# max-andr/joint-cnn-mrf

Hardware: AMD Instinct MI355X
Metric: images/sec (720x480, K=9 joints) part-detector+spatial-model fwd (higher is better)
Workload: dtype f32(fp16x2 spectra, fft); 1 GPU; configs[1]: batch=64/GPU synthetic 480x720x3, part detector + spatial model forward + argmax, fp32; batch_per_gpu=64, global_batch=64, micro_batch=64, use_sm=True, collective=all_gather coords int32 [B,2,9]

## Files before the change

### joint-cnn-mrf_amd/csrc/conv_fft.hip

```cpp
#include <cmath>
#include <cstdlib>
#include <map>
#include <mutex>
#include <utility>
#include <vector>

#include "conv_fft_common.h"

namespace jcm {
namespace cfft {

template <int KS, int NP>
__global__ __launch_bounds__(256) void weight_spectra_split_kernel(const float* __restrict__ w, uint4* __restrict__ Ws, int Cin, int Cout, int CoutP, int ntl, int NY, int NX,
                                                                   int round_bf16, float* __restrict__ wscale) {
  __shared__ cf twy[192][KS - 1], twx[KS];
  const int tid = threadIdx.x;
  const int kx = blockIdx.y;
#pragma unroll 1
  for (int k = tid; k < NY * (KS - 1) + KS; k += 256) {
    const bool isy = k < NY * (KS - 1);
    const int ky = k / (KS - 1), a = isy ? k % (KS - 1) + 1 : k - NY * (KS - 1);
    const int num = isy ? (ky * a) % NY : (kx * a) % NX, den = isy ? NY : NX;
    double sn, cs;
    sincospi(-2.0 * (double)num / (double)den, &sn, &cs);
    cf* dstw = isy ? &twy[ky][a - 1] : &twx[a];
    *dstw = cf{(float)cs, (float)sn};
  }
  __syncthreads();
  constexpr int CPT = 8;
  constexpr int NPP = NP == 5 ? 1 : 2;
  static_assert(NP == 2 || NP == 4 || NP == 5, "operand forms of the channel GEMM");
  float wmul = 1.f;
  if constexpr (NP >= 4) {
    int ex = 0;
    const float bound = wscale[0];
    if (bound > 0.f && bound < 3.0e38f) (void)frexpf(bound, &ex);
    wmul = ldexpf(1.f, 14 - ex);
    if (blockIdx.x == 0 && blockIdx.y == 0 && threadIdx.x == 0) wscale[1] = ldexpf(1.f, ex - 14);
  }
  const size_t e = (size_t)blockIdx.x * 256 + tid;
  if (e >= (size_t)(Cin / CPT) * CoutP) return;
  const int co = (int)(e % CoutP), cig = (int)(e / CoutP);
  cf ra[CPT][KS];
  const unsigned toff = (unsigned)(cig * CPT * Cout + (co < Cout ? co : Cout - 1));
#pragma unroll
  for (int c = 0; c < CPT; ++c)
#pragma unroll
    for (int a = 0; a < KS; ++a) ra[c][a] = cf{0.f, 0.f};
#pragma unroll 1
  for (int a = 0; a < KS; ++a) {
    cf sum[CPT];
#pragma unroll
    for (int c = 0; c < CPT; ++c) sum[c] = cf{0.f, 0.f};
#pragma unroll
    for (int b = 0; b < KS; ++b) {
      const float* tap = w + (size_t)((KS - 1 - a) * KS + (KS - 1 - b)) * Cin * Cout;
      const cf tw = twx[b];
#pragma unroll
      for (int c = 0; c < CPT; ++c) {
        float wv = tap[toff + (unsigned)(c * Cout)];
        wv = co < Cout ? wv : 0.f;
        if (round_bf16) wv = static_cast<float>(static_cast<__bf16>(wv));
        sum[c] = sfma(wv, tw, sum[c]);
      }
    }
#pragma unroll
    for (int c = 0; c < CPT; ++c)
#pragma unroll
      for (int aa = 0; aa < KS; ++aa) ra[c][aa] = aa == a ? sum[c] : ra[c][aa];
  }
  const int KC = Cin / 16, ntiles = CoutP / ntl;
  const int ci0 = cig * CPT, kc = ci0 >> 4, kg = (ci0 >> 3) & 1, nt = co / ntl, sn = co % ntl;
  const size_t fstride = NP == 5 ? (size_t)ntiles * (KC >> 1) * 8 * ntl : (size_t)ntiles * KC * (4 * NPP) * ntl;
  uint4* dst = Ws + (size_t)kx * NY * fstride +
               (NP == 5 ? ((size_t)nt * (KC >> 1) + (kc >> 1)) * 8 * ntl + ((size_t)(kc & 1) * 2 + kg) * ntl + sn :
                          ((size_t)nt * KC + kc) * (4 * NPP) * ntl + (size_t)kg * ntl + sn);
  typedef unsigned u32x4n __attribute__((ext_vector_type(4)));
  auto put = [](uint4* q, const uint4& v) __attribute__((always_inline)) { __builtin_nontemporal_store(u32x4n{v.x, v.y, v.z, v.w}, reinterpret_cast<u32x4n*>(q)); };
  auto emit = [&](uint4* d, const float (&xr)[CPT], const float (&xi)[CPT]) __attribute__((always_inline)) {
    if constexpr (NP == 5) {
      float x8[8];
#pragma unroll
      for (int c = 0; c < 8; ++c) x8[c] = xr[c % CPT];
      put(d, round8h(x8, wmul));
#pragma unroll
      for (int c = 0; c < 8; ++c) x8[c] = xi[c % CPT];
      put(d + (size_t)4 * ntl, round8h(x8, wmul));
    } else {
      uint4 u[NPP];
      float x8[8];
#pragma unroll
      for (int c = 0; c < 8; ++c) x8[c] = xr[c % CPT];
      if constexpr (NP == 4) split8h(x8, wmul, u);
      else split8<NPP>(x8, u);
#pragma unroll
      for (int p = 0; p < NPP; ++p) put(d + (size_t)p * 2 * ntl, u[p]);
#pragma unroll
      for (int c = 0; c < 8; ++c) x8[c] = xi[c % CPT];
      if constexpr (NP == 4) split8h(x8, wmul, u);
      else split8<NPP>(x8, u);
#pragma unroll
      for (int p = 0; p < NPP; ++p) put(d + (size_t)(NPP + p) * 2 * ntl, u[p]);
    }
  };
  for (int ky = 0; ky <= NY / 2; ++ky) {
    const int kp = ky == 0 ? 0 : NY - ky;
    float cs[KS - 1], sn_[KS - 1];
#pragma unroll
    for (int a = 1; a < KS; ++a) { const cf t = twy[ky][a - 1]; cs[a - 1] = t.x; sn_[a - 1] = -t.y; }
    float xr[CPT], xi[CPT], pr[CPT], pi_[CPT];
#pragma unroll
    for (int c = 0; c < CPT; ++c) {
      cf C = ra[c][0], S = cf{0.f, 0.f};
#pragma unroll
      for (int a = 1; a < KS; ++a) { C = sfma(cs[a - 1], ra[c][a], C); S = sfma(sn_[a - 1], ra[c][a], S); }
      xr[c] = C.x + S.y; xi[c] = C.y - S.x;
      pr[c] = C.x - S.y; pi_[c] = C.y + S.x;
    }
    emit(dst + (size_t)ky * fstride, xr, xi);
    if (kp != ky) emit(dst + (size_t)kp * fstride, pr, pi_);
  }
}

template <int TAPS>
__global__ __launch_bounds__(256) void weight_bound_kernel(const float* __restrict__ w, size_t pairs, int round_bf16, float* __restrict__ wmax) {
  __shared__ float red[4];
  float m = 0.f;
  for (size_t e = (size_t)blockIdx.x * 256 + threadIdx.x; e < pairs; e += (size_t)gridDim.x * 256) {
    float v[TAPS];
#pragma unroll
    for (int t = 0; t < TAPS; ++t) v[t] = w[(size_t)t * pairs + e];
    float sum = 0.f;
#pragma unroll
    for (int t = 0; t < TAPS; ++t) {
      float x = v[t];
      if (round_bf16) x = static_cast<float>(static_cast<__bf16>(x));
      sum += fabsf(x);
    }
    m = fmaxf(m, sum);
  }
  block_max_to<256>(m * 1.0001f, wmax, red, threadIdx.x);
}

struct Sizes { int NY, NX; };
static const int kLens[] = {20, 24, 28, 32, 36, 40, 50, 60, 64, 72, 96, 100, 128, 192};
static bool pick(int need, int* n) {
  for (int v : kLens)
    if (v >= need) { *n = v; return true; }
  return false;
}
static int tw_offset(int n) {
  int off = 0;
  for (int v : kLens) {
    if (v == n) return off;
    off += v;
  }
  return -1;
}
static bool sizes_of(int H, int W, int ks, Sizes* s, int circ = 0) {
  if (circ) {
    s->NY = H; s->NX = W;
    return (ks == 9 || ks == 5) && H > 8 && W > 8 && tw_offset(H) >= 0 && tw_offset(W) >= 0;
  }
  return (ks == 9 || ks == 5) && H + ks - 1 <= 192 && W + ks - 1 <= 192 && pick(H + 4, &s->NY) && pick(W + 4, &s->NX);
}
static int pad64(int c) { return (c + CB - 1) / CB * CB; }
static bool fft_reg_on() {
  static const bool on = [] { const char* e = std::getenv("JCM_FFT_REG"); return !e || std::atoi(e) != 0; }();
  return on;
}
static bool fft_tiles_on() {
  static const bool on = [] { const char* e = std::getenv("JCM_FFT_TILES"); return !e || std::atoi(e) != 0; }();
  return on;
}
static int padn(int c, int n) { return (c + n - 1) / n * n; }

int persistent_grid(const void* kernel, int ntiles, int threads, int dyn_lds) {
  static std::mutex mu;
  static std::map<std::pair<const void*, int>, int> cache;
  int dev = 0;
  (void)hipGetDevice(&dev);
  int resident = 0;
  {
    std::lock_guard<std::mutex> lk(mu);
    auto it = cache.find({kernel, dev});
    if (it != cache.end()) resident = it->second;
  }
  if (!resident) {
    int ncu = 256, per_cu = 0;
    (void)hipDeviceGetAttribute(&ncu, hipDeviceAttributeMultiprocessorCount, dev);
    if (hipOccupancyMaxActiveBlocksPerMultiprocessor(&per_cu, kernel, threads, (size_t)dyn_lds) != hipSuccess || per_cu < 1) per_cu = 1;
    resident = ncu * per_cu;
    std::lock_guard<std::mutex> lk(mu);
    cache[{kernel, dev}] = resident;
  }
  return resident < ntiles ? resident : ntiles;
}

static const cf* twiddle_table(int dev) {
  static std::mutex mu;
  static std::map<int, cf*> tabs;
  std::lock_guard<std::mutex> lk(mu);
  auto it = tabs.find(dev);
  if (it != tabs.end()) return it->second;
  std::vector<float> h;
  for (int n : kLens)
    for (int k = 0; k < n; ++k) {
      const double ang = 2.0 * 3.14159265358979323846 * (double)k / (double)n;
      h.push_back((float)std::cos(ang));
      h.push_back((float)std::sin(ang));
    }
  cf* d = nullptr;
  if (hipMalloc(reinterpret_cast<void**>(&d), h.size() * sizeof(float)) != hipSuccess) return nullptr;
  if (hipMemcpy(d, h.data(), h.size() * sizeof(float), hipMemcpyHostToDevice) != hipSuccess) { (void)hipFree(d); return nullptr; }
  tabs[dev] = d;
  return d;
}

}

using namespace cfft;

bool conv_fft_supported(const ConvArgs& a, int ks) {
  Sizes s;
  return a.Cin % CB == 0 && a.Cin >= CB && a.Cout >= 1 && a.B >= 1 && sizes_of(a.H, a.W, ks, &s, a.circ);
}
size_t conv_fft_weight_bytes(int H, int W, int ks, int Cin, int Cout, int np, int circ) {
  Sizes s;
  if (!sizes_of(H, W, ks, &s, circ)) return 0;
  return cgemm_split_w_bytes(np, s.NY * (s.NX / 2 + 1), Cin, Cout);
}
hipError_t conv_fft_pack_weights(const float* w_hwio, void* wf, int H, int W, int ks, int Cin, int Cout, int np, bool round_bf16, hipStream_t st, float* wscale, int circ,
                                 const float* bound_from) {
  Sizes s;
  if (!sizes_of(H, W, ks, &s, circ) || Cin % 16 || (np != 2 && np != 4 && np != 5) || (np >= 4 && !wscale) || (np == 5 && Cin % 32)) return hipErrorInvalidValue;
  const int ntl = cgemm_split_ntile(np, Cout), CoutP = padn(Cout, ntl);
  const size_t cpt = 8;
  const dim3 grid((unsigned)(((size_t)Cin / cpt * CoutP + 255) / 256), (unsigned)(s.NX / 2 + 1));
  uint4* dst = static_cast<uint4*>(wf);
  const int rb = round_bf16 ? 1 : 0;
  if (np >= 4 && bound_from) {
    if (hipError_t e = hipMemcpyAsync(wscale, bound_from, sizeof(float), hipMemcpyDeviceToDevice, st); e != hipSuccess) return e;
  } else if (np >= 4) {
    if (hipError_t e = hipMemsetAsync(wscale, 0, 2 * sizeof(float), st); e != hipSuccess) return e;
    const size_t pairs = (size_t)Cin * Cout;
    const dim3 bgrid((unsigned)((pairs + 255) / 256 > 1024 ? 1024 : (pairs + 255) / 256));
    if (ks == 9) hipLaunchKernelGGL(weight_bound_kernel<81>, bgrid, dim3(256), 0, st, w_hwio, pairs, rb, wscale);
    else hipLaunchKernelGGL(weight_bound_kernel<25>, bgrid, dim3(256), 0, st, w_hwio, pairs, rb, wscale);
  }
#define WS_LAUNCH(KS, NPV) hipLaunchKernelGGL((weight_spectra_split_kernel<KS, NPV>), grid, dim3(256), 0, st, w_hwio, dst, Cin, Cout, CoutP, ntl, s.NY, s.NX, rb, wscale)
  if (ks == 9) {
    if (np == 2) WS_LAUNCH(9, 2); else if (np == 4) WS_LAUNCH(9, 4); else WS_LAUNCH(9, 5);
  } else {
    if (np == 2) WS_LAUNCH(5, 2); else if (np == 4) WS_LAUNCH(5, 4); else WS_LAUNCH(5, 5);
  }
#undef WS_LAUNCH
  return hipGetLastError();
}
namespace {
struct Plan3 { size_t t_bytes, xs_bytes, yf_bytes, sc_fwd_bytes, sc_inv_bytes; int MT, NXH, F, ldy, inv_cb; };
Plan3 plan_of(const ConvArgs& a, const Sizes& s, int np) {
  Plan3 p;
  p.NXH = s.NX / 2 + 1;
  p.F = s.NY * p.NXH;
  p.ldy = padn(a.Cout, cgemm_split_ntile(np, a.Cout));
  if (p.ldy < pad64(a.Cout)) p.ldy = pad64(a.Cout);
  p.MT = cgemm_split_mtile(np, a.B, a.Cout);
  const size_t cop = pad64(a.Cout), cmax = (size_t)a.Cin > cop ? a.Cin : cop;
  const size_t bp = (size_t)(a.B + p.MT - 1) / p.MT * p.MT;
  p.t_bytes = (size_t)a.B * p.NXH * a.H * cmax * sizeof(cf);
  p.xs_bytes = (size_t)p.F * bp * a.Cin * 4 * cgemm_split_parts(np);
  p.yf_bytes = (size_t)p.F * a.B * p.ldy * sizeof(cf);
  p.inv_cb = s.NY > 100 ? 32 : 64;
  p.sc_fwd_bytes = (size_t)a.B * a.H * (a.Cin / CB) * sizeof(float);
  p.sc_inv_bytes = (size_t)a.B * p.NXH * (cop / p.inv_cb) * sizeof(float);
  return p;
}
size_t align256(size_t v) { return (v + 255) & ~size_t(255); }
ConvArgs tile_view(const ConvArgs& a, const Sizes& s) {
  ConvArgs t = a;
  t.B = 4 * a.B; t.H = s.NY; t.W = a.W / 2;
  t.tiles = 0;
  return t;
}
}
size_t conv_fft_workspace_bytes(const ConvArgs& a, int ks, int np) {
  Sizes s;
  if (!(a.tiles ? sizes_of(a.H / 2, a.W / 2, ks, &s) : sizes_of(a.H, a.W, ks, &s, a.circ))) return 0;
  const Plan3 p = a.tiles ? plan_of(tile_view(a, s), s, np) : plan_of(a, s, np);
  return align256(p.t_bytes) + align256(p.xs_bytes) + align256(p.yf_bytes) + align256(p.sc_fwd_bytes) + align256(p.sc_inv_bytes);
}
bool conv_fft_fusable(const ConvArgs& a, int ks, int ks_next) {
  Sizes s, n;
  return sizes_of(a.H, a.W, ks, &s) && sizes_of(a.H, a.W, ks_next, &n) && s.NX == n.NX && a.Cout % CB == 0;
}
size_t conv_fft_handover_bytes(const ConvArgs& a, int ks) {
  Sizes s;
  if (!sizes_of(a.H, a.W, ks, &s)) return 0;
  return (size_t)a.B * (s.NX / 2 + 1) * a.H * a.Cout * sizeof(cf);
}
bool conv_fft_win_gather_supported(int win, int Cin) { return fft_reg_on() && cfft_rows_fwd_win_reg_supported(win, Cin); }
bool conv_fft_win_scatter_supported(int win, int Cout) { return fft_reg_on() && win == 32 && Cout % 64 == 0; }
bool conv_fft_pool_fusable(const ConvArgs& a, int ks, int ks_next) {
  Sizes s, n;
  return sizes_of(a.H, a.W, ks, &s) && sizes_of((a.H + 1) / 2, (a.W + 1) / 2, ks_next, &n) && cfft_rows_inv_pool_fwd_supported(s.NX, n.NX, a.Cout);
}
size_t conv_fft_pool_handover_bytes(const ConvArgs& a, int ks_next) {
  Sizes n;
  if (!sizes_of((a.H + 1) / 2, (a.W + 1) / 2, ks_next, &n)) return 0;
  return (size_t)a.B * (n.NX / 2 + 1) * ((a.H + 1) / 2) * a.Cout * sizeof(cf);
}
bool conv_fft_tiles_supported(const ConvArgs& a, int ks, int ks_next) {
  Sizes s;
  return fft_reg_on() && fft_tiles_on() && ks == 5 && ks_next == 5 && !a.circ && !a.win_map && a.B >= 1 && conv_fft_pool_fusable(a, ks, ks_next) &&
         a.H % 4 == 0 && a.W % 4 == 0 && sizes_of(a.H / 2, a.W / 2, ks, &s) && cfft_tiles_supported(s.NY, s.NX, a);
}
bool conv_fft_merge_fusable(const ConvArgs& a, int ks, int ks_next, const FftMerge& m, bool h16) {
  Sizes s;
  if (!conv_fft_fusable(a, ks, ks_next) || !sizes_of(a.H, a.W, ks, &s)) return false;
  const bool reg = fft_reg_on() && cfft_rows_inv_merge_fwd_reg_supported(s.NX, a, m, (ks - 1) / 2);
  return h16 ? reg : (reg || cfft_rows_inv_merge_fwd_supported(s.NX, a, m));
}
static hipError_t conv_fft_tiles_f32(const ConvArgs& a0, int ks, int np, int in_layout, void* work, const void* t_in, void* t_next, const FftMerge* merge,
                                     hipEvent_t g0, hipEvent_t g1, hipStream_t st, void* xs, bool xs_ready, const Fp16Scale* scp, const FftNext* nx) {
  Sizes s;
  if (np != 4 || in_layout != 0 || t_in || merge || xs || xs_ready || !t_next || !nx || !nx->pool || nx->merge || !scp || !scp->tmax || !scp->winv || !scp->tmax_next ||
      !conv_fft_tiles_supported(a0, ks, nx->ks_next) || !sizes_of(a0.H / 2, a0.W / 2, ks, &s))
    return hipErrorInvalidValue;
  ConvArgs a = a0;
  a.CoutP = pad64(a.Cout);
  const ConvArgs at = tile_view(a, s);
  const Plan3 p = plan_of(at, s, np);
  Fp16Scale sc = *scp;
  sc.hf = (float)s.NY;
  sc.nb = at.B;
  char* wk = static_cast<char*>(work);
  cf* T = reinterpret_cast<cf*>(wk);
  void* Xs = wk + align256(p.t_bytes);
  cf* Yf = reinterpret_cast<cf*>(wk + align256(p.t_bytes) + align256(p.xs_bytes));
  int dev = 0;
  if (hipError_t e = hipGetDevice(&dev); e != hipSuccess) return e;
  const cf* twb = twiddle_table(dev);
  if (!twb) return hipErrorOutOfMemory;
  if (!cfft_rows_fwd_tile_reg(s.NY, s.NX, a, T, sc.tmax, st)) return hipErrorInvalidValue;
  if (hipError_t ce = cfft_cols_fwd(s.NY, at, np, T, Xs, twb + tw_offset(s.NY), p.NXH, p.MT, sc, st); ce != hipSuccess) return ce;
  if (hipError_t e = hipGetLastError(); e != hipSuccess) return e;
  if (g0 && hipEventRecord(g0, st) != hipSuccess) return hipErrorUnknown;
  if (hipError_t e = cgemm_split(Xs, a.wp, Yf, np, p.F, at.B, a.Cin, a.Cout, p.ldy, st, 0.f); e != hipSuccess) return e;
  if (g1 && hipEventRecord(g1, st) != hipSuccess) return hipErrorUnknown;
  ConvArgs ai = at;
  ai.H = a.H / 2;
  if (!cfft_cols_inv_reg(s.NY, ai, Yf, T, p.NXH, p.ldy, (ks - 1) / 2, st, nullptr, 0.f)) return hipErrorInvalidValue;
  if (!cfft_rows_inv_pool_tile_reg(s.NY, s.NX, a, T, static_cast<cf*>(t_next), 1.0f / (float)(s.NY * s.NX), sc, st)) return hipErrorInvalidValue;
  return hipGetLastError();
}
hipError_t conv_fft_f32(const ConvArgs& a0, int ks, int np, int in_layout, int out_layout, void* work, const void* t_in, void* t_next, const FftMerge* merge,
                        hipEvent_t g0, hipEvent_t g1, hipStream_t st, void* xs, bool xs_ready, const Fp16Scale* scp, const FftNext* nx) {
  if (a0.tiles) return conv_fft_tiles_f32(a0, ks, np, in_layout, work, t_in, t_next, merge, g0, g1, st, xs, xs_ready, scp, nx);
  Sizes s;
  if (!conv_fft_supported(a0, ks) || !sizes_of(a0.H, a0.W, ks, &s, a0.circ) || (out_layout == 2 && a0.Cout % 8) || (np != 2 && np != 4 && np != 5) || (np == 5 && a0.Cin % 32)) return hipErrorInvalidValue;
  if (a0.circ && (t_in || t_next || merge || in_layout != 0 || out_layout != 0)) return hipErrorInvalidValue;
  if (nx && (nx->pool || nx->merge) && (!t_next || (nx->pool && nx->merge))) return hipErrorInvalidValue;
  Fp16Scale sc;
  if (np >= 4) {
    if (!scp || !scp->tmax || !scp->winv || (t_next && !scp->tmax_next)) return hipErrorInvalidValue;
    sc = *scp;
    sc.hf = (float)a0.H;
    sc.nb = a0.B;
  }
  const bool h16 = sc.t16 && ((t_next && nx && nx->merge && !t_in) || (t_in && !t_next));
  if ((t_in || t_next) && !h16 && (in_layout != 0 || out_layout != 0)) return hipErrorInvalidValue;
  if (t_next && a0.Cout % CB) return hipErrorInvalidValue;
  if (sc.t16 && (np != 5 || in_layout == 0 || out_layout == 0 || xs || ((t_in || t_next) && !h16))) return hipErrorInvalidValue;
  if (merge && in_layout == 2) return hipErrorInvalidValue;
  ConvArgs a = a0;
  a.CoutP = pad64(a.Cout);
  const int opad = (ks - 1) / 2 + (a0.circ ? 4 : 0);
  const Plan3 p = plan_of(a, s, np);
  char* wk = static_cast<char*>(work);
  cf* T = reinterpret_cast<cf*>(wk);
  void* Xs = xs ? xs : wk + align256(p.t_bytes);
  cf* Yf = reinterpret_cast<cf*>(wk + align256(p.t_bytes) + align256(p.xs_bytes));
  if (sc.t16) {
    sc.t16_fwd = reinterpret_cast<float*>(wk + align256(p.t_bytes) + align256(p.xs_bytes) + align256(p.yf_bytes));
    sc.t16_inv = reinterpret_cast<float*>(wk + align256(p.t_bytes) + align256(p.xs_bytes) + align256(p.yf_bytes) + align256(p.sc_fwd_bytes));
    sc.t16_cb = p.inv_cb;
    if (t_in) sc.t16_fwd = reinterpret_cast<float*>(const_cast<char*>(static_cast<const char*>(t_in)) + align256((size_t)a.B * p.NXH * a.H * a.Cin * 4));
  }
  if (xs_ready && !xs) return hipErrorInvalidValue;
  int dev = 0;
  if (hipError_t e = hipGetDevice(&dev); e != hipSuccess) return e;
  const cf* twb = twiddle_table(dev);
  if (!twb) return hipErrorOutOfMemory;
  const cf* twx = twb + tw_offset(s.NX);
  const cf* twy = twb + tw_offset(s.NY);
  const float norm = 1.0f / (float)(s.NY * s.NX);
  const cf* Tin = t_in ? static_cast<const cf*>(t_in) : T;
  const bool fft_reg = fft_reg_on();
  if (!xs_ready) {
    if (merge && !t_in) {
      if (!(fft_reg && cfft_rows_fwd_merge_reg(s.NX, a, *merge, in_layout, T, sc.tmax, st, sc.t16_fwd))) cfft_rows_fwd_merge(s.NX, a, *merge, in_layout, T, twx, sc.tmax, st, sc.t16_fwd);
    } else if (!t_in) {
      if (a.win_map) { if (!cfft_rows_fwd_win_reg(s.NX, a, T, sc.tmax, st)) return hipErrorInvalidValue; }
      else if (!(fft_reg && cfft_rows_fwd_reg(s.NX, a, in_layout, T, sc.tmax, st, sc.t16_fwd))) cfft_rows_fwd(s.NX, a, in_layout, T, twx, sc.tmax, st, sc.t16_fwd);
    }
    if (hipError_t ce = cfft_cols_fwd(s.NY, a, np, Tin, Xs, twy, p.NXH, p.MT, sc, st); ce != hipSuccess) return ce;
  }
  if (hipError_t e = hipGetLastError(); e != hipSuccess) return e;
  if (g0 && hipEventRecord(g0, st) != hipSuccess) return hipErrorUnknown;
  const float yshift = sc.t16 ? cgemm_split_y16_shift(a.Cin) : 0.f, yinv = yshift != 0.f ? 1.0f / yshift : 0.f;
  if (hipError_t e = cgemm_split(Xs, a.wp, Yf, np, p.F, a.B, a.Cin, a.Cout, p.ldy, st, yshift); e != hipSuccess) return e;
  if (g1 && hipEventRecord(g1, st) != hipSuccess) return hipErrorUnknown;
  ConvArgs ai = a;
  if (a0.circ) { ai.H = a0.H - 8; ai.W = a0.W - 8; }
  if (!(fft_reg && p.inv_cb == 64 && cfft_cols_inv_reg(s.NY, ai, Yf, T, p.NXH, p.ldy, opad, st, sc.t16_inv, yinv))) cfft_cols_inv(s.NY, ai, Yf, T, twy, p.NXH, p.ldy, opad, st, sc.t16_inv, yinv);
  if (t_next && nx && nx->pool) {
    Sizes sn;
    if (!sizes_of((a.H + 1) / 2, (a.W + 1) / 2, nx->ks_next, &sn) ||
        !cfft_rows_inv_pool_fwd(s.NX, sn.NX, a, T, static_cast<cf*>(t_next), twx, twb + tw_offset(sn.NX), opad, norm, sc, st))
      return hipErrorInvalidValue;
  } else if (t_next && nx && nx->merge) {
    if (sc.t16) {
      float* t16n = reinterpret_cast<float*>(static_cast<char*>(t_next) + align256((size_t)a.B * p.NXH * a.H * a.Cout * 4));
      if (!(fft_reg && cfft_rows_inv_merge_fwd_reg(s.NX, a, *nx->merge, T, static_cast<cf*>(t_next), opad, norm, sc, st, t16n))) return hipErrorInvalidValue;
    } else if (!(fft_reg && cfft_rows_inv_merge_fwd_reg(s.NX, a, *nx->merge, T, static_cast<cf*>(t_next), opad, norm, sc, st)) &&
               !cfft_rows_inv_merge_fwd(s.NX, a, *nx->merge, T, static_cast<cf*>(t_next), twx, opad, norm, sc, st)) {
      return hipErrorInvalidValue;
    }
  } else if (t_next) {
    if (!(fft_reg && cfft_rows_inv_fwd_reg(s.NX, a, T, static_cast<cf*>(t_next), opad, norm, sc, st))) cfft_rows_inv_fwd(s.NX, a, T, static_cast<cf*>(t_next), twx, opad, norm, sc, st);
  } else if (!((ai.rows_mfma & 1) && cfft_rows_inv_mfma(s.NX, ai, out_layout, T, opad, norm, sc, st)) && !(fft_reg && cfft_rows_inv_reg(s.NX, ai, out_layout, T, opad, norm, sc, st))) {
    if (ai.wout_TX > 0) return hipErrorInvalidValue;
    cfft_rows_inv(s.NX, ai, out_layout, T, twx, opad, norm, sc, st);
  }
  return hipGetLastError();
}

size_t conv_fft_xs_bytes(const ConvArgs& a, int ks, int np) {
  Sizes s;
  if (!sizes_of(a.H, a.W, ks, &s, a.circ)) return 0;
  return align256(plan_of(a, s, np).xs_bytes);
}
hipError_t conv_fft_spectra(const ConvArgs& a0, int ks, int np, void* work, void* xs, hipStream_t st, float* tmax, int common) {
  Sizes s;
  if (!conv_fft_supported(a0, ks) || !sizes_of(a0.H, a0.W, ks, &s, a0.circ) || !xs || (np >= 4 && !tmax)) return hipErrorInvalidValue;
  Fp16Scale sc;
  if (np >= 4) { sc.tmax = tmax; sc.hf = (float)a0.H; sc.nb = a0.B; sc.common = common; }
  ConvArgs a = a0;
  a.CoutP = pad64(a.Cout);
  const Plan3 p = plan_of(a, s, np);
  int dev = 0;
  if (hipError_t e = hipGetDevice(&dev); e != hipSuccess) return e;
  const cf* twb = twiddle_table(dev);
  if (!twb) return hipErrorOutOfMemory;
  cf* T = static_cast<cf*>(work);
  if (a.win_map) { if (!cfft_rows_fwd_win_reg(s.NX, a, T, sc.tmax, st)) return hipErrorInvalidValue; }
  else cfft_rows_fwd(s.NX, a, 0, T, twb + tw_offset(s.NX), sc.tmax, st);
  if (hipError_t ce = cfft_cols_fwd(s.NY, a, np, T, xs, twb + tw_offset(s.NY), p.NXH, p.MT, sc, st); ce != hipSuccess) return ce;
  return hipGetLastError();
}
bool conv_fft_geometry(int H, int W, int ks, int B, int Cout, int np, int* NY, int* NX, int* MT, int circ) {
  Sizes s;
  if (!sizes_of(H, W, ks, &s, circ)) return false;
  *NY = s.NY; *NX = s.NX; *MT = cgemm_split_mtile(np, B, Cout);
  return true;
}

}
```

### joint-cnn-mrf_amd/csrc/conv_fft_cols.hip

```cpp
#include "conv_fft_common.h"

namespace jcm {
namespace cfft {

template <int NY, int NP, bool T16 = false>
__global__ __launch_bounds__(colfwd_threads<NY>()) void cols_fwd_split_kernel(const cf* __restrict__ T, uint4* __restrict__ Xs, const cf* __restrict__ twg, int B, int H, int KC, int MT,
                                                            int mtiles, const float* __restrict__ tmax, int common, const float* __restrict__ t16, int ntiles) {
  constexpr int IMG = colimg<NY>(), CH = IMG * 16, NTC = colfwd_threads<NY>(), NPP = NP == 5 ? 1 : 2;
  constexpr int CPV = T16 ? 4 : 2;
  constexpr int NV = NY * CH / CPV, KV = (NV + NTC - 1) / NTC, VPR = CH / CPV, VPI = 16 / CPV;
  extern __shared__ __attribute__((aligned(16))) char smem_cf[];
  cf* buf = reinterpret_cast<cf*>(smem_cf);
  cf* tw = buf + NY * CH;
  float4* buf4 = reinterpret_cast<float4*>(buf);
  const int tid = threadIdx.x;
  const int NG = (B + IMG - 1) / IMG;
  twiddles<NY, NTC>(tw, twg, tid);
  __shared__ float xsc[IMG];
  uint4 pre[KV];
  float psc[KV];
  auto coords = [&](int tile, int& kc, int& kx, int& b0, int& nimg) __attribute__((always_inline)) {
    const int g = tile % NG, kk = tile / NG;
    kc = kk % KC; kx = kk / KC;
    b0 = g * IMG; nimg = min(IMG, B - b0);
  };
  auto prefetch = [&](int tile) __attribute__((always_inline)) {
    int kc, kx, b0, nimg;
    coords(tile, kc, kx, b0, nimg);
    const uint4* src = reinterpret_cast<const uint4*>(T) + (((size_t)kx * KC + kc) * B + b0) * H * VPI;
#pragma unroll
    for (int i = 0; i < KV; ++i) {
      const int t = tid + i * NTC, y = t / VPR, v = t % VPR, img = v / VPI, cv = v % VPI;
      const bool ok = t < NV && y < H && img < nimg;
      pre[i] = ok ? src[((size_t)img * H + y) * VPI + cv] : make_uint4(0u, 0u, 0u, 0u);
      if constexpr (T16) psc[i] = ok ? t16[((size_t)(b0 + img) * (KC >> 2) + (kc >> 2)) * H + y] : 0.f;
    }
  };
  int tile = blockIdx.x;
  if (tile < ntiles) prefetch(tile);
  for (; tile < ntiles; tile += gridDim.x) {
    int kc, kx, b0, nimg;
    coords(tile, kc, kx, b0, nimg);
#pragma unroll
    for (int i = 0; i < KV; ++i) {
      const int t = tid + i * NTC;
      if (t < NV) {
        if constexpr (T16) {
          const cf a = unpack_h2(pre[i].x, psc[i]), b2 = unpack_h2(pre[i].y, psc[i]), c2 = unpack_h2(pre[i].z, psc[i]), d2 = unpack_h2(pre[i].w, psc[i]);
          buf4[2 * t] = make_float4(a.x, a.y, b2.x, b2.y);
          buf4[2 * t + 1] = make_float4(c2.x, c2.y, d2.x, d2.y);
        } else {
          buf4[t] = make_float4(__uint_as_float(pre[i].x), __uint_as_float(pre[i].y), __uint_as_float(pre[i].z), __uint_as_float(pre[i].w));
        }
      }
    }
    if constexpr (NP >= 4)
      if (tid < IMG) xsc[tid] = tid < nimg ? fp16_scale(tmax_of(tmax, b0 + tid, B, common), (float)H) : 1.f;
    __syncthreads();
    if (tile + (int)gridDim.x < ntiles) prefetch(tile + (int)gridDim.x);
    fft<NY, -1, CH, NTC>(buf, tw, tid);
    const int mt = b0 / MT, r0 = b0 - mt * MT;
    for (int it = tid; it < NY * 2 * IMG; it += NTC) {
      const int img = it % IMG, kg = (it / IMG) & 1, ky = it / (2 * IMG);
      const cf* z = buf + pos<NY>(ky) * CH + img * 16 + kg * 8;
      float re[8], im[8];
#pragma unroll
      for (int e = 0; e < 8; ++e) { re[e] = z[e].x; im[e] = z[e].y; }
      uint4 ur[NPP], ui[NPP];
      if constexpr (NP == 5) {
        const float xscale = xsc[img];
        ur[0] = round8h(re, xscale);
        ui[0] = round8h(im, xscale);
      } else if constexpr (NP == 4) {
        const float xscale = xsc[img];
        split8h(re, xscale, ur);
        split8h(im, xscale, ui);
      } else {
        split8<NPP>(re, ur);
        split8<NPP>(im, ui);
      }
      const size_t f = (size_t)kx * NY + ky;
      if constexpr (NP == 5) {
        uint4* dst = Xs + (((f * mtiles + mt) * (KC >> 1) + (kc >> 1)) * 8 + (size_t)(kc & 1) * 2 + kg) * MT + r0 + img;
        st_stream(dst, ur[0]);
        st_stream(dst + (size_t)4 * MT, ui[0]);
      } else {
        uint4* dst = Xs + (((f * mtiles + mt) * KC + kc) * (4 * NPP) + kg) * MT + r0 + img;
#pragma unroll
        for (int p = 0; p < NPP; ++p) {
          st_stream(dst + (size_t)(0 * NPP + p) * 2 * MT, ur[p]);
          st_stream(dst + (size_t)(1 * NPP + p) * 2 * MT, ui[p]);
        }
      }
    }
    __syncthreads();
  }
}

template <int NY, bool T16 = false>
__global__ __launch_bounds__(colinv_threads<NY>()) void cols_inv_kernel(const cf* __restrict__ Yf, cf* __restrict__ T, const cf* __restrict__ twg, int B, int H, int NXH, int C, int ldy,
                                                      int pad, float* __restrict__ t16, float yinv) {
  constexpr int CH = colblk<NY>(), CB = CH, NTC = colinv_threads<NY>();
  __shared__ cf buf[NY * CH];
  __shared__ cf tw[NY];
  const int tid = threadIdx.x;
  const int cblk = blockIdx.x % (C / CB), bk = blockIdx.x / (C / CB);
  const int kx = bk % NXH, b = bk / NXH;
  twiddles<NY, NTC>(tw, twg, tid);
  for (int t = tid; t < NY * CH; t += NTC) {
    const int ky = t / CH, v = t % CH;
    const size_t src = ((size_t)(kx * NY + ky) * B + b) * ldy + cblk * CB + v;
    if constexpr (T16) buf[t] = unpack_h2(reinterpret_cast<const unsigned*>(Yf)[src], 1.f);
    else buf[t] = Yf[src];
  }
  __syncthreads();
  fft<NY, 1, CH, NTC>(buf, tw, tid);
  if constexpr (T16) {
    constexpr int KM = (NY * CH + NTC - 1) / NTC;
    __shared__ float red[NTC / 64];
    cf val[KM];
    float m = 0.f;
#pragma unroll
    for (int i = 0; i < KM; ++i) {
      const int t = tid + i * NTC, y = t / CH, v = t % CH;
      val[i] = cf{0.f, 0.f};
      if (t < H * CH) {
        val[i] = buf[pos<NY>(y + pad) * CH + v];
        m = fmaxf(m, fmaxf(fabsf(val[i].x), fabsf(val[i].y)));
      }
    }
    const float s = bfp_scale(block_max_all<NTC>(m, red, tid));
    unsigned* dst = reinterpret_cast<unsigned*>(T);
#pragma unroll
    for (int i = 0; i < KM; ++i) {
      const int t = tid + i * NTC, y = t / CH, v = t % CH;
      if (t < H * CH) st_stream(&dst[((size_t)(b * H + y) * NXH + kx) * C + cblk * CB + v], pack_h2(val[i].x * s, val[i].y * s));
    }
    if (tid == 0) t16[((size_t)b * (C / CB) + cblk) * NXH + kx] = (1.0f / s) * yinv;
  } else {
    for (int t = tid; t < H * CH; t += NTC) {
      const int y = t / CH, v = t % CH;
      st_stream(&T[((size_t)(b * H + y) * NXH + kx) * C + cblk * CB + v], buf[pos<NY>(y + pad) * CH + v]);
    }
  }
}


template <int NY> static hipError_t launch_cols_fwd(const ConvArgs& a, int np, const cf* T, void* Xs, const cf* tw, int NXH, int MT, const Fp16Scale& sc, hipStream_t st) {
  constexpr int IMG = colimg<NY>();
  constexpr int lds = (NY * IMG * 16 + NY) * (int)sizeof(cf);
  const int KC = a.Cin / 16, mtiles = (a.B + MT - 1) / MT;
  const int ntiles = NXH * KC * ((a.B + IMG - 1) / IMG);
  static LdsAttr attr2, attr4, attr5, attr5h;
  const dim3 blk(colfwd_threads<NY>());
#define COLS_FWD(KERNEL, ATTR, ...)                                                                              \
  do {                                                                                                           \
    if (hipError_t e = ATTR.ensure(reinterpret_cast<const void*>(KERNEL), lds); e != hipSuccess) return e;        \
    const dim3 grid((unsigned)persistent_grid(reinterpret_cast<const void*>(KERNEL), ntiles, (int)blk.x, lds));  \
    hipLaunchKernelGGL(KERNEL, grid, blk, lds, st, T, static_cast<uint4*>(Xs), tw, a.B, a.H, KC, MT, mtiles, __VA_ARGS__, ntiles); \
  } while (0)
  if (np == 5 && sc.t16_fwd) {
    if (!sc.tmax || (KC & 3)) return hipErrorInvalidValue;
    COLS_FWD((cols_fwd_split_kernel<NY, 5, true>), attr5h, sc.tmax, sc.common, sc.t16_fwd);
  } else if (np == 5) {
    if (!sc.tmax || (KC & 1)) return hipErrorInvalidValue;
    COLS_FWD((cols_fwd_split_kernel<NY, 5>), attr5, sc.tmax, sc.common, (const float*)nullptr);
  } else if (np == 2) {
    COLS_FWD((cols_fwd_split_kernel<NY, 2>), attr2, (const float*)nullptr, 0, (const float*)nullptr);
  } else if (np == 4) {
    if (!sc.tmax) return hipErrorInvalidValue;
    COLS_FWD((cols_fwd_split_kernel<NY, 4>), attr4, sc.tmax, sc.common, (const float*)nullptr);
  } else {
    return hipErrorInvalidValue;
  }
#undef COLS_FWD
  return hipSuccess;
}
template <int NY> static void launch_cols_inv(const ConvArgs& a, const cf* Yf, cf* T, const cf* tw, int NXH, int ldy, int pad, hipStream_t st, float* t16, float y16_inv) {
  const dim3 grid(a.B * NXH * (a.CoutP / colblk<NY>())), blk(colinv_threads<NY>());
  if (t16) hipLaunchKernelGGL((cols_inv_kernel<NY, true>), grid, blk, 0, st, Yf, T, tw, a.B, a.H, NXH, a.CoutP, ldy, pad, t16, y16_inv);
  else hipLaunchKernelGGL((cols_inv_kernel<NY, false>), grid, blk, 0, st, Yf, T, tw, a.B, a.H, NXH, a.CoutP, ldy, pad, nullptr, 0.f);
}
hipError_t cfft_cols_fwd(int NY, const ConvArgs& a, int np, const cf* T, void* Xs, const cf* tw, int NXH, int MT, const Fp16Scale& sc, hipStream_t st) {
  hipError_t e = hipSuccess;
#define CALL(N) e = launch_cols_fwd<N>(a, np, T, Xs, tw, NXH, MT, sc, st)
  CFFT_BY_SIZE(NY, CALL)
#undef CALL
  return e;
}
void cfft_cols_inv(int NY, const ConvArgs& a, const cf* Yf, cf* T, const cf* tw, int NXH, int ldy, int pad, hipStream_t st, float* t16, float y16_inv) {
#define CALL(N) launch_cols_inv<N>(a, Yf, T, tw, NXH, ldy, pad, st, t16, y16_inv)
  CFFT_BY_SIZE(NY, CALL)
#undef CALL
}

}
}
```

### joint-cnn-mrf_amd/csrc/conv_fft_common.h

```cpp
#pragma once
#include "fft_lds.h"
#include "kernels.h"

namespace jcm {
namespace cfft {
using namespace fftl;
constexpr int CB = 64, NT = 256;
constexpr int kParMax = 512;

template <int N> struct Plan;
template <> struct Plan<192> { static constexpr int R1 = 8, R2 = 8, R3 = 3; };
template <> struct Plan<128> { static constexpr int R1 = 8, R2 = 4, R3 = 4; };
template <> struct Plan<100> { static constexpr int R1 = 4, R2 = 5, R3 = 5; };
template <> struct Plan<96> { static constexpr int R1 = 8, R2 = 12, R3 = 1; };
template <> struct Plan<72> { static constexpr int R1 = 8, R2 = 3, R3 = 3; };
template <> struct Plan<64> { static constexpr int R1 = 8, R2 = 8, R3 = 1; };
template <> struct Plan<60> { static constexpr int R1 = 4, R2 = 15, R3 = 1; };
template <> struct Plan<50> { static constexpr int R1 = 5, R2 = 10, R3 = 1; };
template <> struct Plan<40> { static constexpr int R1 = 8, R2 = 5, R3 = 1; };
template <> struct Plan<36> { static constexpr int R1 = 4, R2 = 3, R3 = 3; };
template <> struct Plan<32> { static constexpr int R1 = 8, R2 = 4, R3 = 1; };
template <> struct Plan<28> { static constexpr int R1 = 4, R2 = 7, R3 = 1; };
template <> struct Plan<24> { static constexpr int R1 = 8, R2 = 3, R3 = 1; };
template <> struct Plan<20> { static constexpr int R1 = 4, R2 = 5, R3 = 1; };
// ... 84 lines not shown
  return ((((size_t)k * (C >> 4) + cblk * 4 + (v >> 3)) * B + b) * H + y) * 8 + (v & 7);
}
template <int NX, int NTH = NT>
__device__ __forceinline__ float rows_fwd_store(const cf* buf, cf* __restrict__ T, int tid, int cblk, int b, int y, int B, int H, int C) {
  constexpr int CH = CB / 2, NXH = NX / 2 + 1;
  float4* dst = reinterpret_cast<float4*>(T);
  float m = 0.f;
  for (int t = tid; t < NXH * CH; t += NTH) {
    const int k = t / CH, v = t % CH;
    const cf zk = buf[pos<NX>(k) * CH + v], zn = buf[pos<NX>(k == 0 ? 0 : NX - k) * CH + v];
    const float4 o = make_float4(0.5f * (zk.x + zn.x), 0.5f * (zk.y - zn.y), 0.5f * (zk.y + zn.y), -0.5f * (zk.x - zn.x));
    dst[t_fwd_index(k, cblk, v, b, y, B, H, C)] = o;
    m = fmaxf(fmaxf(m, fmaxf(fabsf(o.x), fabsf(o.y))), fmaxf(fabsf(o.z), fabsf(o.w)));
  }
  return m;
}

template <int NX, int NTH = NT>
__device__ __forceinline__ float rows_fwd_store16(const cf* buf, void* T, float* __restrict__ tinv, float* red2, int tid, int cblk, int b, int y, int B, int H, int C) {
  constexpr int CH = CB / 2, NXH = NX / 2 + 1, K = (NXH * CH + NTH - 1) / NTH;
  uint2* dst = reinterpret_cast<uint2*>(T);
  float4 o[K];
  float m = 0.f;
#pragma unroll
  for (int i = 0; i < K; ++i) {
    const int t = tid + i * NTH, k = t / CH, v = t % CH;
    o[i] = make_float4(0.f, 0.f, 0.f, 0.f);
    if (t < NXH * CH) {
      const cf zk = buf[pos<NX>(k) * CH + v], zn = buf[pos<NX>(k == 0 ? 0 : NX - k) * CH + v];
      o[i] = make_float4(0.5f * (zk.x + zn.x), 0.5f * (zk.y - zn.y), 0.5f * (zk.y + zn.y), -0.5f * (zk.x - zn.x));
      m = fmaxf(fmaxf(m, fmaxf(fabsf(o[i].x), fabsf(o[i].y))), fmaxf(fabsf(o[i].z), fabsf(o[i].w)));
    }
  }
  const float s = bfp_scale(block_max_all<NTH>(m, red2, tid));
#pragma unroll
  for (int i = 0; i < K; ++i) {
    const int t = tid + i * NTH, k = t / CH, v = t % CH;
    if (t < NXH * CH) dst[t_fwd_index(k, cblk, v, b, y, B, H, C)] = make_uint2(pack_h2(o[i].x * s, o[i].y * s), pack_h2(o[i].z * s, o[i].w * s));
  }
  if (tid == 0) tinv[((size_t)b * (C / CB) + cblk) * H + y] = 1.0f / s;
  return m;
}

constexpr int kFp16TargetExp = 15;
static_assert(kFp16TargetExp <= 15, "sqrt(2) * 2^kFp16TargetExp must stay below fp16's largest number 65504");
__device__ __forceinline__ int fp16_exp(float tmax, float hf) {
  const float bound = tmax * hf;
  int e = 0;
  if (bound > 0.f && bound < 3.0e38f) (void)frexpf(bound, &e);
  return e;
}
__device__ __forceinline__ int fp16_k(float tmax, float hf) { const int k = kFp16TargetExp - fp16_exp(tmax, hf); return k > 126 ? 126 : (k < -126 ? -126 : k); }
__device__ __forceinline__ float fp16_scale(float tmax, float hf) { return ldexpf(1.f, fp16_k(tmax, hf)); }
__device__ __forceinline__ float fp16_unscale(float tmax, float hf) { return ldexpf(1.f, -fp16_k(tmax, hf)); }
__device__ __forceinline__ float tmax_of(const float* __restrict__ tmax, int b, int nb, int common) {
  if (!common) return tmax[b];
  float m = 0.f;
  for (int i = 0; i < nb; ++i) m = fmaxf(m, tmax[i]);
  return m;
}
__device__ __forceinline__ void wave_max_stash(float m, float* red) {
#pragma unroll
  for (int o = 32; o > 0; o >>= 1) m = fmaxf(m, __shfl_xor(m, o));
  if ((threadIdx.x & 63) == 0) red[threadIdx.x >> 6] = m;
}
template <int NTH>
__device__ __forceinline__ void stash_to_word(const float* red, float* dst) {
  if (threadIdx.x == 0) {
    float m = red[0];
#pragma unroll
    for (int w = 1; w < NTH / 64; ++w) m = fmaxf(m, red[w]);
    if (m > 0.f) atomicMax(reinterpret_cast<unsigned*>(dst), __float_as_uint(m));
  }
}
template <int NTH>
__device__ __forceinline__ void block_max_to(float m, float* dst, float* red, int tid) {
#pragma unroll
  for (int o = 32; o > 0; o >>= 1) m = fmaxf(m, __shfl_xor(m, o));
  if ((tid & 63) == 0) red[tid >> 6] = m;
  __syncthreads();
  if (tid == 0) {
    for (int w = 1; w < NTH / 64; ++w) m = fmaxf(m, red[w]);
    if (m > 0.f) atomicMax(reinterpret_cast<unsigned*>(dst), __float_as_uint(m));
  }
}
template <int NX> constexpr int rows_threads() { return NX >= 128 ? 512 : NX >= 72 ? 384 : 256; }
template <int NY> constexpr int colblk() { return NY > 100 ? 32 : 64; }
template <int NY> constexpr int colimg() { return NY > 96 ? 4 : 8; }
template <int NY> constexpr int colfwd_threads() { return NY * colimg<NY>() * 16 >= 8192 ? 1024 : NY * colimg<NY>() * 16 >= 4096 ? 512 : 256; }
template <int NY> constexpr int colinv_threads() { return NY * colblk<NY>() >= 4096 ? 512 : 256; }
__device__ __forceinline__ void split8h(const float (&x)[8], float scale, uint4 (&out)[2]) {
  unsigned short h[2][8];
#pragma unroll
  for (int e = 0; e < 8; ++e) {
    float v = x[e] * scale;
#pragma unroll
    for (int p = 0; p < 2; ++p) {
      const _Float16 q = static_cast<_Float16>(v);
      h[p][e] = __builtin_bit_cast(unsigned short, q);
      v = v - static_cast<float>(q);
    }
  }
#pragma unroll
  for (int p = 0; p < 2; ++p)
    out[p] = make_uint4((unsigned)h[p][0] | ((unsigned)h[p][1] << 16), (unsigned)h[p][2] | ((unsigned)h[p][3] << 16), (unsigned)h[p][4] | ((unsigned)h[p][5] << 16),
                        (unsigned)h[p][6] | ((unsigned)h[p][7] << 16));
}
__device__ __forceinline__ uint4 round8h(const float (&x)[8], float scale) {
  unsigned short h[8];
#pragma unroll
  for (int e = 0; e < 8; ++e) h[e] = __builtin_bit_cast(unsigned short, static_cast<_Float16>(x[e] * scale));
  return make_uint4((unsigned)h[0] | ((unsigned)h[1] << 16), (unsigned)h[2] | ((unsigned)h[3] << 16), (unsigned)h[4] | ((unsigned)h[5] << 16), (unsigned)h[6] | ((unsigned)h[7] << 16));
}
template <int NP>
__device__ __forceinline__ void split8(const float (&x)[8], uint4 (&out)[NP]) {
  unsigned short h[NP][8];
#pragma unroll
  for (int e = 0; e < 8; ++e) {
    float v = x[e];
#pragma unroll
    for (int p = 0; p < NP; ++p) {
      const __bf16 q = static_cast<__bf16>(v);
      h[p][e] = __builtin_bit_cast(unsigned short, q);
      v = v - static_cast<float>(q);
    }
  }
#pragma unroll
  for (int p = 0; p < NP; ++p)
    out[p] = make_uint4((unsigned)h[p][0] | ((unsigned)h[p][1] << 16), (unsigned)h[p][2] | ((unsigned)h[p][3] << 16), (unsigned)h[p][4] | ((unsigned)h[p][5] << 16),
                        (unsigned)h[p][6] | ((unsigned)h[p][7] << 16));
}
#define CFFT_BY_SIZE(N, CALL)                    \
  switch (N) {                                   \
    case 20: CALL(20); break;                    \
    case 24: CALL(24); break;                    \
    case 28: CALL(28); break;                    \
    case 32: CALL(32); break;                    \
    case 36: CALL(36); break;                    \
    case 40: CALL(40); break;                    \
    case 50: CALL(50); break;                    \
    case 60: CALL(60); break;                    \
    case 64: CALL(64); break;                    \
    case 72: CALL(72); break;                    \
    case 96: CALL(96); break;                    \
    case 100: CALL(100); break;                  \
    case 128: CALL(128); break;                  \
    default: CALL(192); break;                   \
  }

int persistent_grid(const void* kernel, int ntiles, int threads, int dyn_lds = 0);

void cfft_rows_fwd(int NX, const ConvArgs& a, int layout, cf* T, const cf* tw, float* tmax, hipStream_t st, float* t16 = nullptr);
void cfft_rows_fwd_merge(int NX, const ConvArgs& a, const FftMerge& m, int in_layout, cf* T, const cf* tw, float* tmax, hipStream_t st, float* t16 = nullptr);
hipError_t cfft_cols_fwd(int NY, const ConvArgs& a, int np, const cf* T, void* Xs, const cf* tw, int NXH, int MT, const Fp16Scale& sc, hipStream_t st);
void cfft_cols_inv(int NY, const ConvArgs& a, const cf* Yf, cf* T, const cf* tw, int NXH, int ldy, int pad, hipStream_t st, float* t16 = nullptr, float y16_inv = 0.f);
void cfft_rows_inv(int NX, const ConvArgs& a, int layout, const cf* T, const cf* tw, int pad, float norm, const Fp16Scale& sc, hipStream_t st);
bool cfft_rows_inv_reg(int NX, const ConvArgs& a, int layout, const cf* T, int pad, float norm, const Fp16Scale& sc, hipStream_t st);
bool cfft_rows_inv_fwd_reg(int NX, const ConvArgs& a, const cf* T, cf* Tn, int pad, float norm, const Fp16Scale& sc, hipStream_t st);
bool cfft_rows_fwd_reg(int NX, const ConvArgs& a, int layout, cf* T, float* tmax, hipStream_t st, float* t16);
bool cfft_rows_fwd_win_reg(int NX, const ConvArgs& a, cf* T, float* tmax, hipStream_t st);
bool cfft_rows_fwd_win_reg_supported(int NX, int Cin);
bool cfft_tiles_supported(int NY, int NX, const ConvArgs& a);
bool cfft_rows_fwd_tile_reg(int NY, int NX, const ConvArgs& a, cf* T, float* tmax, hipStream_t st);
bool cfft_rows_inv_pool_tile_reg(int NY, int NX, const ConvArgs& a, const cf* T, cf* Tn, float norm, const Fp16Scale& sc, hipStream_t st);
bool cfft_rows_fwd_merge_reg(int NX, const ConvArgs& a, const FftMerge& m, int in_layout, cf* T, float* tmax, hipStream_t st, float* t16);
bool cfft_cols_inv_reg(int NY, const ConvArgs& a, const cf* Yf, cf* T, int NXH, int ldy, int pad, hipStream_t st, float* t16, float y16_inv = 0.f);
void cfft_rows_inv_fwd(int NX, const ConvArgs& a, const cf* T, cf* Tn, const cf* tw, int pad, float norm, const Fp16Scale& sc, hipStream_t st);
bool cfft_rows_inv_pool_fwd(int NXI, int NXO, const ConvArgs& a, const cf* T, cf* Tn, const cf* twi, const cf* two, int pad, float norm, const Fp16Scale& sc, hipStream_t st);
bool cfft_rows_inv_merge_fwd(int NX, const ConvArgs& a, const FftMerge& m, const cf* T, cf* Tn, const cf* tw, int pad, float norm, const Fp16Scale& sc, hipStream_t st);
bool cfft_rows_inv_merge_fwd_reg(int NX, const ConvArgs& a, const FftMerge& m, const cf* T, cf* Tn, int pad, float norm, const Fp16Scale& sc, hipStream_t st, float* t16n = nullptr);
bool cfft_rows_inv_merge_fwd_reg_supported(int NX, const ConvArgs& a, const FftMerge& m, int pad);
bool cfft_rows_inv_pool_fwd_supported(int NXI, int NXO, int Cout);
bool cfft_rows_inv_mfma(int NX, const ConvArgs& a, int layout, const cf* T, int pad, float norm, const Fp16Scale& sc, hipStream_t st);
bool cfft_rows_inv_merge_fwd_supported(int NX, const ConvArgs& a, const FftMerge& m);
}
}
```

### joint-cnn-mrf_amd/csrc/conv_fft_rows_reg.hip

```cpp
#include <type_traits>

#include "conv_fft_common.h"
#include "fft_reg.h"
#include "resize_tf1.h"

namespace jcm {
namespace cfft {
using namespace fftr;

template <int NX, int K1, bool ALL = false, class St>
__device__ __forceinline__ void inv_rows_out2(const cf (&u)[NX / 2], int h, int W, int pad, St&& store) {
  constexpr int M = NX / 2, R1 = RPlan<M>::R1, R2 = RPlan<M>::R2;
  cf o[R2];
  step2_row<M, 1, K1>(u, o);
#pragma unroll
  for (int k2 = 0; k2 < R2; ++k2) {
    const int xo = 2 * (K1 + R1 * k2) + h - pad;
    if (ALL || (xo >= 0 && xo < W)) store(K1 + R1 * k2, xo, o[k2]);
  }
  __builtin_amdgcn_sched_barrier(0);
  if constexpr (K1 + 1 < R1) inv_rows_out2<NX, K1 + 1, ALL>(u, h, W, pad, store);
}
template <int NX, int N>
__device__ __forceinline__ void inv_rows_in2(cf (&u)[NX / 2], const float4& q1, const float4& q2, float sg, bool odd) {
// ... 65 lines not shown
      typedef float f4 __attribute__((ext_vector_type(4)));
      const f4 q = __builtin_bit_cast(f4, __builtin_amdgcn_raw_buffer_load_b128(d, vo, k * ko, 0));
      return make_float4(q[0], q[1], q[2], q[3]);
    };
    inv_rows_load2<NX, T16, 0>(u, sg, odd, load);
  }
  float norm = norm0;
  if (sc.tmax) {
    float tm;
    if (sc.common) {
      tm = 0.f;
      for (int i = (int)(threadIdx.x & 63); i < sc.nb; i += 64) tm = fmaxf(tm, sc.tmax[i]);
#pragma unroll
      for (int o = 32; o > 0; o >>= 1) tm = fmaxf(tm, __shfl_xor(tm, o));
    } else {
      tm = sc.tmax[b];
    }
    norm = norm0 * sc.winv[0] * fp16_unscale(tm, sc.hf);
  }
  const bool two = c + 1 < Cout;
  float b0v = 0.f, b1v = 0.f, s0 = 1.f, s1 = 1.f, h0 = 0.f, h1 = 0.f;
  if (c < Cout) {
    b0v = bias[c];
    if (two) b1v = bias[c + 1];
    if (relu_bn) { s0 = scale[c]; h0 = shift[c]; if (two) { s1 = scale[c + 1]; h1 = shift[c + 1]; } }
  }
  step1<M, 1>(u);
  const int lane = threadIdx.x & 63;
  int sc_row = -1, sc_x0 = 0;
  if (LAYOUT == 0 && sTX > 0) {
    const int bw = (int)(by / H), yv = (int)(by % H);
    const int tx = bw % sTX, ty = (bw / sTX) % sTY, bi = bw / (sTX * sTY), ym = ty * H + yv;
    sc_row = ym < smH ? bi * smH + ym : -1;
    sc_x0 = tx * W;
  }
  unsigned* wst = stage + (LAYOUT != 0 ? (threadIdx.x >> 6) * (M * 64) : 0);
  auto store = [&](int m, int xo, cf z) __attribute__((always_inline)) {
    float v0 = fmaf(z.x, norm, b0v), v1 = fmaf(z.y, norm, b1v);
    if (relu_bn) { v0 = fmaf(fmaxf(v0, 0.f), s0, h0); v1 = fmaf(fmaxf(v1, 0.f), s1, h1); }
    if constexpr (LAYOUT == 0) {
      if (sTX > 0) {
        const int xm = sc_x0 + xo;
        if (sc_row >= 0 && xm < smW) st_stream(reinterpret_cast<cf*>(static_cast<float*>(out) + ((size_t)sc_row * smW + xm) * Cout + c), cf{v0, v1});
      } else {
        st_stream(reinterpret_cast<cf*>(static_cast<float*>(out) + (by * W + xo) * Cout + c), cf{v0, v1});
      }
    } else {
      typedef __bf16 bf16x2 __attribute__((ext_vector_type(2)));
      wst[(m * 2 + h) * 32 + (lane >> 1)] = __builtin_bit_cast(unsigned, bf16x2{static_cast<__bf16>(v0), static_cast<__bf16>(v1)});
    }
  };
  if (two || LAYOUT != 0) inv_rows_out2<NX, 0, LAYOUT != 0>(u, h, W, pad, store);
  if constexpr (LAYOUT != 0) {
    __builtin_amdgcn_fence(__ATOMIC_RELEASE, "wavefront");
    __builtin_amdgcn_wave_barrier();
    const int y = (int)(by % H);
    const int c0 = c - (lane >> 1) * 2;
    const uint4* rd = reinterpret_cast<const uint4*>(wst);
#pragma unroll 4
    for (int q = lane; q < M * 16; q += 64) {
      const int m = q >> 4, hh = (q >> 3) & 1, j = q & 7;
      const int xo = 2 * m + hh - pad, cu = c0 + 8 * j;
      if (xo >= 0 && xo < W && cu < Cout) {
        __bf16* o = LAYOUT == 1 ? static_cast<__bf16*>(out) + (by * W + xo) * Cout + cu
                                : static_cast<__bf16*>(out) + (((size_t)b * (Cout >> 3) + (cu >> 3)) * H * W + (size_t)y * W + xo) * 8;
        *reinterpret_cast<uint4*>(o) = rd[q];
      }
    }
  }
}

template <int NY, int K1>
__device__ __forceinline__ void inv_cols_rows(cf (&x)[NY]) {
  constexpr int R1 = RPlan<NY>::R1, R2 = RPlan<NY>::R2;
  cf o[R2];
  step2_row<NY, 1, K1>(x, o);
#pragma unroll
  for (int k2 = 0; k2 < R2; ++k2) x[R2 * K1 + k2] = o[k2];
  if constexpr (K1 + 1 < R1) inv_cols_rows<NY, K1 + 1>(x);
}
__device__ __forceinline__ unsigned lane_pair_swap(unsigned w) { return (unsigned)__builtin_amdgcn_mov_dpp((int)w, 0xB1, 0xF, 0xF, true); }
template <int NY, bool T16>
__global__ __launch_bounds__(256) __attribute__((amdgpu_waves_per_eu(NY >= 64 ? 2 : 3, NY >= 64 ? 2 : 8))) void cols_inv_reg_kernel(const cf* __restrict__ Yf, void* __restrict__ T, int B, int H, int NXH, int C, int ldy,
                                                                                              int pad, float* __restrict__ t16, float yinv) {
  static_assert(NY % 2 == 0, "ky pairs");
  constexpr int R1 = RPlan<NY>::R1, R2 = RPlan<NY>::R2;
  const size_t g = (size_t)blockIdx.x * 256 + threadIdx.x;
  const int c = (int)(g % C);
  const unsigned bk = (unsigned)__builtin_amdgcn_readfirstlane((int)(g / C));
  const int kx = (int)(bk % (unsigned)NXH), b = (int)(bk / (unsigned)NXH);
  if (b >= B) return;
  const bool odd = (c & 1) != 0;
  cf x[NY];
  if constexpr (T16) {
    const uint2* src = reinterpret_cast<const uint2*>(reinterpret_cast<const unsigned*>(Yf) + ((size_t)kx * NY * B + b) * ldy + (c & ~1));
    const size_t kstep = (size_t)B * ldy / 2;
    uint2 raw[NY / 2];
#pragma unroll
    for (int i = 0; i < NY / 2; ++i) raw[i] = src[(size_t)(2 * i + (odd ? 1 : 0)) * kstep];
    __builtin_amdgcn_sched_barrier(0);
#pragma unroll
    for (int i = 0; i < NY / 2; ++i) {
      const unsigned keep = odd ? raw[i].y : raw[i].x, recv = lane_pair_swap(odd ? raw[i].x : raw[i].y);
      x[2 * i] = unpack_h2(odd ? recv : keep, 1.f);
      x[2 * i + 1] = unpack_h2(odd ? keep : recv, 1.f);
    }
  } else {
    const cf* src = Yf + ((size_t)kx * NY * B + b) * ldy + c;
#pragma unroll
    for (int ky = 0; ky < NY; ++ky) x[ky] = src[(size_t)ky * B * ldy];
  }
  step1<NY, 1>(x);
  inv_cols_rows<NY, 0>(x);
  if constexpr (T16) {
    float m = 0.f;
#pragma unroll
    for (int i = 0; i < NY; ++i) {
      const int y = (i / R2) + R1 * (i % R2) - pad;
      if (y >= 0 && y < H) m = fmaxf(m, fmaxf(fabsf(x[i].x), fabsf(x[i].y)));
    }
#pragma unroll
    for (int o = 32; o > 0; o >>= 1) m = fmaxf(m, __shfl_xor(m, o));
    const float s = bfp_scale(m);
    if ((threadIdx.x & 63) == 0) t16[((size_t)b * (C >> 6) + (c >> 6)) * NXH + kx] = (1.0f / s) * yinv;
    uint2* dst = reinterpret_cast<uint2*>(reinterpret_cast<unsigned*>(T) + ((size_t)b * H * NXH + kx) * C + (c & ~1));
    const size_t ystep = (size_t)NXH * C / 2;
#pragma unroll
    for (int k = 0; k < NY; k += 2) {
      const int ia = R2 * (k % R1) + k / R1, ib = R2 * ((k + 1) % R1) + (k + 1) / R1;
      const unsigned va = pack_h2(x[ia].x * s, x[ia].y * s), vb = pack_h2(x[ib].x * s, x[ib].y * s);
      const unsigned recv = lane_pair_swap(odd ? va : vb);
      const int y = k - pad + (odd ? 1 : 0);
      if (y >= 0 && y < H) st_stream(dst + (size_t)y * ystep, make_uint2(odd ? recv : va, odd ? vb : recv));
    }
  } else {
#pragma unroll
    for (int i = 0; i < NY; ++i) {
      const int y = (i / R2) + R1 * (i % R2) - pad;
      if (y >= 0 && y < H) st_stream(reinterpret_cast<cf*>(T) + ((size_t)(b * H + y) * NXH + kx) * C + c, x[i]);
    }
  }
}
bool cfft_cols_inv_reg(int NY, const ConvArgs& a, const cf* Yf, cf* T, int NXH, int ldy, int pad, hipStream_t st, float* t16, float y16_inv) {
  if (a.CoutP % 64 || ((y16_inv != 0.f) != (t16 != nullptr)) || (t16 && ldy % 2)) return false;
  const size_t threads = (size_t)a.B * NXH * a.CoutP;
  const dim3 grid((unsigned)((threads + 255) / 256)), blk(256);
#define CI_LAUNCH(N)                                                                                                                                             \
  do {                                                                                                                                                           \
    if (t16) hipLaunchKernelGGL((cols_inv_reg_kernel<N, true>), grid, blk, 0, st, Yf, static_cast<void*>(T), a.B, a.H, NXH, a.CoutP, ldy, pad, t16, y16_inv);            \
    else hipLaunchKernelGGL((cols_inv_reg_kernel<N, false>), grid, blk, 0, st, Yf, static_cast<void*>(T), a.B, a.H, NXH, a.CoutP, ldy, pad, nullptr, 0.f);          \
  } while (0)
  switch (NY) {
    case 64: CI_LAUNCH(64); break;
    case 36: CI_LAUNCH(36); break;
    case 32: CI_LAUNCH(32); break;
    case 20: CI_LAUNCH(20); break;
    default: return false;
  }
#undef CI_LAUNCH
  return true;
}

__device__ __forceinline__ unsigned pair_word(unsigned w, bool odd) {
  const auto r = __builtin_amdgcn_permlane32_swap(w, w, false, false);
  return odd ? r[0] : r[1];
}
__device__ __forceinline__ void pair_coords(int CP, int& h, int& p, size_t& by) {
  const size_t g = (size_t)blockIdx.x * 256 + threadIdx.x;
  const int lane = threadIdx.x & 63;
  const size_t q = (g >> 6) * 32;
  h = lane >> 5;
  p = (int)((q + (lane & 31)) % CP);
  by = (size_t)(unsigned)__builtin_amdgcn_readfirstlane((int)(q / CP));
}
template <int NX, int J>
__device__ __forceinline__ void fwd_rows_in2(cf (&u)[NX / 2], const unsigned (&raw)[NX / 2], float sg, bool odd) {
  constexpr int M = NX / 2;
  const unsigned oth = pair_word(raw[J], odd);
  const cf a = bf16pair(raw[J]), o = bf16pair(oth);
  cf v = cf{fmaf(sg, a.x, o.x), fmaf(sg, a.y, o.y)};
  if constexpr (J > 0) {
    const float wr = odd ? Tw<-J, NX>::re : 1.f, wi = odd ? Tw<-J, NX>::im : 0.f;
    v = cf{fmaf(-v.y, wi, v.x * wr), fmaf(v.x, wi, v.y * wr)};
  }
  u[J] = v;
  if constexpr (J + 1 < M) fwd_rows_in2<NX, J + 1>(u, raw, sg, odd);
}
template <int N, int S, int K1>
__device__ __forceinline__ void step2_inplace(cf (&x)[N]) {
  constexpr int R1 = RPlan<N>::R1, R2 = RPlan<N>::R2;
  cf o[R2];
  step2_row<N, S, K1>(x, o);
#pragma unroll
  for (int k2 = 0; k2 < R2; ++k2) x[R2 * K1 + k2] = o[k2];
  if constexpr (K1 + 1 < R1) step2_inplace<N, S, K1 + 1>(x);
}
template <int NX, int MI, class F>
__device__ __forceinline__ void fwd_rows_visit(const cf (&u)[NX / 2], bool odd, F&& f) {
  constexpr int M = NX / 2, R1 = RPlan<M>::R1, R2 = RPlan<M>::R2;
  constexpr int m0 = (M - MI) % M, m1 = M - 1 - MI;
  const cf zk = u[R2 * (MI % R1) + MI / R1], za = u[R2 * (m0 % R1) + m0 / R1], zb = u[R2 * (m1 % R1) + m1 / R1];
  const cf zn = cf{odd ? zb.x : za.x, odd ? zb.y : za.y};
  f(MI, make_float4(0.5f * (zk.x + zn.x), 0.5f * (zk.y - zn.y), 0.5f * (zk.y + zn.y), -0.5f * (zk.x - zn.x)));
  if constexpr (2 * (MI + 1) <= M) fwd_rows_visit<NX, MI + 1>(u, odd, f);
}
template <int NX>
__device__ __forceinline__ void fwd_rows_finish(const unsigned (&raw)[NX / 2], uint2* __restrict__ T, int h, int p, int b, int y, int B, int H, int C, float* __restrict__ tmax,
                                                float* __restrict__ t16) {
  constexpr int M = NX / 2;
  const bool odd = h != 0;
  const int lane = threadIdx.x & 63;
  cf u[M];
  fwd_rows_in2<NX, 0>(u, raw, odd ? -1.f : 1.f, odd);
  step1<M, -1>(u);
  step2_inplace<M, -1, 0>(u);
  float m = 0.f;
  fwd_rows_visit<NX, 0>(u, odd, [&](int mi, const float4& o) __attribute__((always_inline)) {
    if (2 * mi + h <= M) m = fmaxf(fmaxf(m, fmaxf(fabsf(o.x), fabsf(o.y))), fmaxf(fabsf(o.z), fabsf(o.w)));
  });
#pragma unroll
  for (int sft = 32; sft > 0; sft >>= 1) m = fmaxf(m, __shfl_xor(m, sft));
  const float sc = bfp_scale(m);
  const int cblk = p >> 5, v = p & 31;
  if (lane == 0) {
    t16[((size_t)b * (C >> 6) + cblk) * H + y] = 1.0f / sc;
    if (tmax && m > 0.f) atomicMax(reinterpret_cast<unsigned*>(tmax + b), __float_as_uint(m));
  }
  uint2* dst = T + ((((size_t)cblk * 4 + (v >> 3)) * B + b) * H + y) * 8 + (v & 7);
  const size_t kstride = (size_t)(C >> 4) * B * H * 8;
  fwd_rows_visit<NX, 0>(u, odd, [&](int mi, const float4& o) __attribute__((always_inline)) {
    const int k = 2 * mi + h;
    if (k <= M) dst[(size_t)k * kstride] = make_uint2(pack_h2(o.x * sc, o.y * sc), pack_h2(o.z * sc, o.w * sc));
  });
}
template <int NX>
__global__ __launch_bounds__(256) __attribute__((amdgpu_waves_per_eu(NX >= 96 ? 3 : 4, NX >= 96 ? 3 : 8))) void rows_fwd_reg_kernel(const unsigned* __restrict__ in, uint2* __restrict__ T, int nrows, int B, int H, int W, int C,
                                                                                              float* __restrict__ tmax, float* __restrict__ t16) {
  constexpr int M = NX / 2;
  const int CP = C >> 1;
  int h, p;
  size_t by;
  pair_coords(CP, h, p, by);
  if (by >= (size_t)nrows) return;
  const int b = (int)(by / H), y = (int)(by % H);
  const unsigned* src = in + (by * W) * CP + p;
  unsigned raw[M];
#pragma unroll
  for (int j = 0; j < M; ++j) {
    const int n = h * M + j;
    raw[j] = n < W ? src[(size_t)n * CP] : 0u;
  }
  fwd_rows_finish<NX>(raw, T, h, p, b, y, B, H, C, tmax, t16);
}
bool cfft_rows_fwd_reg(int NX, const ConvArgs& a, int layout, cf* T, float* tmax, hipStream_t st, float* t16) {
  if ((NX != 96 && NX != 50 && NX != 28) || layout != 1 || !t16 || a.Cin % 64 || a.W > NX) return false;
  const int nrows = a.B * a.H;
  const size_t threads = (size_t)nrows * a.Cin;
  const dim3 grid((unsigned)((threads + 255) / 256)), blk(256);
#define RFR_LAUNCH(N) hipLaunchKernelGGL(rows_fwd_reg_kernel<N>, grid, blk, 0, st, static_cast<const unsigned*>(a.x), reinterpret_cast<uint2*>(T), nrows, a.B, a.H, a.W, a.Cin, tmax, t16)
  if (NX == 96) RFR_LAUNCH(96);
  else if (NX == 50) RFR_LAUNCH(50);
  else RFR_LAUNCH(28);
#undef RFR_LAUNCH
  return true;
}

template <int NX>
__global__ __launch_bounds__(256) void rows_fwd_win_reg_kernel(const float* __restrict__ map, float4* __restrict__ T, int nrows, int BW, int H, int W, int C, int TY, int TX,
                                                               int valid_only, float* __restrict__ tmax) {
  constexpr int NXH = NX / 2 + 1, R1 = RPlan<NX>::R1, R2 = RPlan<NX>::R2, V = NX - 8;
  const int CP = C >> 1;
  const size_t g = (size_t)blockIdx.x * 256 + threadIdx.x;
  const int p = (int)(g % CP);
  const int row = __builtin_amdgcn_readfirstlane((int)(g / CP));
  if (row >= nrows) return;
  const int wy = row % NX, bw = row / NX;
  const int tx = bw % TX, ty = (bw / TX) % TY, b = bw / (TX * TY);
  const int y = ty * V - 4 + wy, x0 = tx * V - 4;
  const bool row_in = y >= 0 && y < H && !(valid_only && (wy < 4 || wy >= NX - 4));
  cf z[NX];
  {
    const auto d = __builtin_amdgcn_make_buffer_rsrc(const_cast<float*>(map) + ((size_t)b * H + (row_in ? y : 0)) * W * C, 0, W * C * 4, 0x00020000);
    typedef float f2 __attribute__((ext_vector_type(2)));
#pragma unroll
    for (int wx = 0; wx < NX; ++wx) {
      const int x = x0 + wx;
      const bool in = row_in && x >= 0 && x < W && !(valid_only && (wx < 4 || wx >= NX - 4));
      z[wx] = cf{0.f, 0.f};
      if (in) z[wx] = __builtin_bit_cast(f2, __builtin_amdgcn_raw_buffer_load_b64(d, p * 8, x * C * 4, 0));
    }
  }
  step1<NX, -1>(z);
  step2_inplace<NX, -1, 0>(z);
  const int cblk = p >> 5, v = p & 31;
  float4* dst = T + ((((size_t)cblk * 4 + (v >> 3)) * BW + bw) * NX + wy) * 8 + (v & 7);
  const size_t kstride = (size_t)(C >> 4) * BW * NX * 8;
  float m = 0.f;
#pragma unroll
  for (int k = 0; k < NXH; ++k) {
    const int kn = k == 0 ? 0 : NX - k;
    const cf zk = z[R2 * (k % R1) + k / R1], zn = z[R2 * (kn % R1) + kn / R1];
    const float4 o = make_float4(0.5f * (zk.x + zn.x), 0.5f * (zk.y - zn.y), 0.5f * (zk.y + zn.y), -0.5f * (zk.x - zn.x));
    dst[(size_t)k * kstride] = o;
    m = fmaxf(fmaxf(m, fmaxf(fabsf(o.x), fabsf(o.y))), fmaxf(fabsf(o.z), fabsf(o.w)));
  }
  if (tmax) {
// ... 665 lines not shown
```

### joint-cnn-mrf_amd/csrc/ctx.h

```cpp
#pragma once
#include "../../include/jcm.h"

#include <map>
#include <mutex>
#include <string>
#include <vector>

#include "kernels.h"

namespace jcm {

struct CallOrder;

int fail(int code, const std::string& msg);

#define HIP_TRY(expr)                                                                                   \
  do {                                                                                                  \
    hipError_t e_ = (expr);                                                                             \
    if (e_ != hipSuccess)                                                                               \
      return ::jcm::fail(JCM_ERR_HIP, std::string(#expr) + ": " + hipGetErrorString(e_));               \
  } while (0)
#define JCM_TRY(expr)          \
  do {                         \
    int r_ = (expr);           \
    if (r_ != JCM_OK) return r_; \
  } while (0)
extern const char* const kJointNames[10];
constexpr int kC = 10;
constexpr float kBnEps = 1e-3f;
constexpr int kHmH = 60, kHmW = 90, kHmHW = kHmH * kHmW;
constexpr int kPrH = 120, kPrW = 180;
constexpr int kCH = 61, kCW = 91;
constexpr size_t kFrame = (size_t)kPrH * kPrW;
constexpr size_t kSpec = (size_t)kPrH * (kPrW / 2 + 1);

struct Tensor {
  std::vector<int64_t> shape;
  float* d = nullptr;
  size_t n = 0;
};

struct ConvLayer {
  int ks = 0, cin = 0, cout = 0, coutp = 0;
  bool has_bn = false;
  const float* w_raw = nullptr;
  float* wp = nullptr;
  mutable bool wp_stale = false;
  void* wp_split = nullptr;
  int coutp_split = 0;
  float* wscale = nullptr;
  void* wp_bf16 = nullptr;
  void* wp_kxfold = nullptr;
  void* wq1_bf16 = nullptr;
  float* wq1_f32 = nullptr;
  void* wq1_split = nullptr;
  int coutp_bf16 = 0;
  bool thin = false;
  bool thin_bf16 = false;
  const float* bias = nullptr;
  float* scale = nullptr;
  float* shift = nullptr;
};

struct TrainState;
}
struct jcm_ctx;
namespace jcm {
void train_destroy(jcm_ctx* c);
const float* train_param_range(jcm_ctx* c, int64_t off, int64_t n);
const double* train_grad_sumsq(jcm_ctx* c);

}

struct jcm_ctx {
  int device = 0;
  hipStream_t stream = nullptr;
  int precision = JCM_PRECISION_F32;
  int K = 9;
  int f32_conv = 0;
  float* act_scale = nullptr;
  float* scale_scratch = nullptr;
  int split_min_wgs = 128;
  bool finalized = false;
  std::map<std::string, jcm::Tensor> params;
  std::map<std::string, jcm::ConvLayer> convs;
  std::vector<void*> owned;
  bool has_sm = false;
  float* sp_energy = nullptr;
  float* sp_bias = nullptr;
  float* bn_sm_scale = nullptr;
  float* bn_sm_shift = nullptr;
  int* cond = nullptr;
  const float** energy_ptrs = nullptr;
  const float** bias_ptrs = nullptr;
  int* cond0 = nullptr;
  int sm_algo = 3;
  void* fft_t_next = nullptr;
  const void* fft_t_in = nullptr;
  void* fft_xs = nullptr;
  bool fft_xs_ready = false;
  void* sm_scratch = nullptr;
  unsigned sm_epoch = 0;
  int fft_tiles = 1;
  int fft_fuse = 3;
  int bf16_hpool = 1;
  int conv_hpool = 0;
  int fft_rows_mfma = 1;
  int fft_next_pool = 0, fft_next_ks = 0;
  const void* fft_win_map = nullptr;
  int fft_win_B = 0, fft_win_H = 0, fft_win_W = 0, fft_win_TY = 0, fft_win_TX = 0;
  bool fft_win_scatter = false;
  bool fft_t_in_16 = false;
  const void* fft_next_merge = nullptr;
  const void* fft_merge = nullptr;
  int conv9_fft = 1;
  int fft_single = 1;
  int fft_win = 1;
  int fft_t16 = 1;
  static constexpr int kFftWords = 1 << 18, kFftWordsPerCall = 1 << 16;
  struct WordBlock { float* p = nullptr; int cap = 0; };
  std::vector<WordBlock> fft_blocks;
  int fft_block_i = 0, fft_word_i = 0;
  int call_order = 1;
  int debug_skip = 0;
  float* fft_tmax_in = nullptr;
  float* fft_last_tmax = nullptr;
  struct FftW { void* p = nullptr; size_t bytes = 0; bool valid = false; float* wscale = nullptr; };
  std::map<std::string, FftW> fft_w;
  int sm_chunk = 32;
  int micro_batch = 0;
  float2* prior_spec_t = nullptr;
  char* arena = nullptr;
  size_t arena_cap = 0, arena_off = 0, arena_peak = 0;
  bool dry = false;
  size_t param_bytes = 0;
  bool profile = false;
  std::map<std::string, std::vector<std::pair<hipEvent_t, hipEvent_t>>> prof;
  std::vector<hipEvent_t> event_pool;
  jcm::TrainState* train = nullptr;
  double* hist_limits = nullptr;
  std::mutex call_mu;
  int call_depth = 0;
  jcm::CallOrder* order = nullptr;
};

namespace jcm {

struct DeviceGuard {
  int prev = -1;
  explicit DeviceGuard(int dev) {
    (void)hipGetDevice(&prev);
    if (prev != dev) (void)hipSetDevice(dev);
    else prev = -1;
  }
  ~DeviceGuard() {
    if (prev >= 0) (void)hipSetDevice(prev);
  }
};

struct CallOrder {
  jcm_ctx* c;
  std::unique_lock<std::mutex> lk;
  std::unique_lock<std::mutex> hlk;
  bool nested = false;
  explicit CallOrder(jcm_ctx* ctx);
  ~CallOrder();
  void acquire();
  void release();
  CallOrder(const CallOrder&) = delete;
  CallOrder& operator=(const CallOrder&) = delete;
};

template <class T>
T* arena_alloc(jcm_ctx* c, size_t count) {
  const size_t bytes = (count * sizeof(T) + 255) & ~size_t(255);
  const size_t off = c->arena_off;
  c->arena_off += bytes;
  if (c->arena_off > c->arena_peak) c->arena_peak = c->arena_off;
  return reinterpret_cast<T*>(c->arena + off);
}

int arena_reserve(jcm_ctx* c, size_t bytes);
int dev_alloc(jcm_ctx* c, void** p, size_t bytes);
int sm_scratch_next(jcm_ctx* c, void** scratch, unsigned* epoch);
const Tensor* find(jcm_ctx* c, const std::string& name);
int check(jcm_handle h, bool need_final);
const ConvLayer* conv_of(jcm_ctx* c, const std::string& scope);
int fold_bn(jcm_ctx* c, const std::string& scope, int n, float** scale, float** shift);
int refresh_derived(jcm_ctx* c, bool first);
int prof_begin(jcm_ctx* c, hipEvent_t* e0, hipEvent_t* e1);
void prof_end(jcm_ctx* c, const std::string& scope, hipEvent_t e0, hipEvent_t e1, bool ok);
void prof_release_all(jcm_ctx* c, bool destroy);
bool takes_fft(jcm_ctx* c, const ConvLayer* L, int B, int H, int W);
bool fft_spectra_valid(jcm_ctx* c, const std::string& scope, int H, int W, int circ = 0);
inline int fft_np(const jcm_ctx* c) { return c->precision == JCM_PRECISION_BF16 ? (c->fft_single ? 5 : 2) : 4; }
int fft_new_words(jcm_ctx* c, int n, float** w);
int run_conv_fft(jcm_ctx* c, const ConvLayer* L, const std::string& scope, const void* x, int B, int H, int W, void* out, int in_layout, int out_layout, int circ = 0);
int run_conv_layer(jcm_ctx* c, const ConvLayer* L, const std::string& scope, int stride, const void* x, int B, int H, int W, int sub,
                   void* out, bool act_bf16, bool out_f32, int in_planar = 0, int out_planar = 0);

inline int cdiv2(int v) { return (v + 1) / 2; }

template <class F>
int with_arena(jcm_ctx* c, F&& body) {
  if (c->call_depth > 1) return fail(JCM_ERR_STATE, "this entry point uses the handle's workspace and cannot be called from the gradient-ready callback of the same handle");
  c->dry = true;
  c->arena_off = 0;
  c->arena_peak = 0;
  int r = body();
  c->dry = false;
  if (r != JCM_OK) return r;
  JCM_TRY(arena_reserve(c, c->arena_peak));
  c->arena_off = 0;
  return body();
}

}
```

### joint-cnn-mrf_amd/csrc/fft_reg.h

```cpp
#pragma once
#include "fft_lds.h"

namespace jcm {
namespace fftr {
using namespace fftl;

constexpr double kPi = 3.14159265358979323846264338327950288;
constexpr double sin_small(double x) {
  double term = x, sum = x;
  for (int i = 1; i < 12; ++i) { term *= -x * x / ((2 * i) * (2 * i + 1)); sum += term; }
  return sum;
}
constexpr double cos_small(double x) {
  double term = 1.0, sum = 1.0;
  for (int i = 1; i < 12; ++i) { term *= -x * x / ((2 * i - 1) * (2 * i)); sum += term; }
  return sum;
}
struct SinCos { double s, c; };
constexpr SinCos sincos_frac(long num, long den) {
  num %= den;
  if (num < 0) num += den;
  const long n8 = num * 8;
  const long o = n8 / den;
  const double r = 2.0 * kPi * (double)(n8 - o * den) / (8.0 * (double)den);
  const double sr = sin_small(r), cr = cos_small(r), h = 0.70710678118654752440084436210485;
  switch (o) {
    case 0: return {sr, cr};
    case 1: return {h * (cr + sr), h * (cr - sr)};
    case 2: return {cr, -sr};
    case 3: return {h * (cr - sr), -h * (cr + sr)};
    case 4: return {-sr, -cr};
    case 5: return {-h * (cr + sr), -h * (cr - sr)};
    case 6: return {-cr, sr};
    default: return {-h * (cr - sr), h * (cr + sr)};
  }
}
template <int NUM, int DEN> struct Tw {
  static constexpr float re = (float)sincos_frac(NUM, DEN).c;
  static constexpr float im = (float)sincos_frac(NUM, DEN).s;
};
template <int NUM, int DEN> __device__ __forceinline__ cf twmul(cf a) {
  constexpr int n = ((NUM % DEN) + DEN) % DEN;
  if constexpr (n == 0) return a;
  else if constexpr (4 * n == DEN) return cf{-a.y, a.x};
  else if constexpr (2 * n == DEN) return cf{-a.x, -a.y};
  else if constexpr (4 * n == 3 * DEN) return cf{a.y, -a.x};
  else {
    constexpr float wr = Tw<n, DEN>::re, wi = Tw<n, DEN>::im;
    return cf{fmaf(-a.y, wi, a.x * wr), fmaf(a.x, wi, a.y * wr)};
  }
}

template <int N> struct RPlan;
template <> struct RPlan<96> { static constexpr int R1 = 8, R2 = 12; };
template <> struct RPlan<64> { static constexpr int R1 = 8, R2 = 8; };
template <> struct RPlan<48> { static constexpr int R1 = 4, R2 = 12; };
template <> struct RPlan<32> { static constexpr int R1 = 4, R2 = 8; };
template <> struct RPlan<16> { static constexpr int R1 = 4, R2 = 4; };
template <> struct RPlan<25> { static constexpr int R1 = 5, R2 = 5; };
template <> struct RPlan<14> { static constexpr int R1 = 2, R2 = 7; };
template <> struct RPlan<50> { static constexpr int R1 = 5, R2 = 10; };
template <> struct RPlan<36> { static constexpr int R1 = 3, R2 = 12; };
template <> struct RPlan<28> { static constexpr int R1 = 4, R2 = 7; };
template <> struct RPlan<20> { static constexpr int R1 = 4, R2 = 5; };

template <int N, int S, int N2, int K1 = 0>
__device__ __forceinline__ void step1_twiddle(cf (&x)[N], const cf (&a)[RPlan<N>::R1]) {
  constexpr int R1 = RPlan<N>::R1, R2 = RPlan<N>::R2;
  x[R2 * K1 + N2] = twmul<S * N2 * K1, N>(a[K1]);
  if constexpr (K1 + 1 < R1) step1_twiddle<N, S, N2, K1 + 1>(x, a);
}
template <int N, int S, int N2 = 0>
__device__ __forceinline__ void step1(cf (&x)[N]) {
  constexpr int R1 = RPlan<N>::R1, R2 = RPlan<N>::R2;
  cf a[R1];
#pragma unroll
  for (int n1 = 0; n1 < R1; ++n1) a[n1] = x[R2 * n1 + N2];
  Dft<R1, S>::run(a);
  step1_twiddle<N, S, N2>(x, a);
  if constexpr (N2 + 1 < R2) step1<N, S, N2 + 1>(x);
}
template <int N, int S, int K1>
__device__ __forceinline__ void step2_row(const cf (&x)[N], cf (&out)[RPlan<N>::R2]) {
  constexpr int R2 = RPlan<N>::R2;
#pragma unroll
  for (int n2 = 0; n2 < R2; ++n2) out[n2] = x[R2 * K1 + n2];
  Dft<R2, S>::run(out);
}

}
}
```

### joint-cnn-mrf_amd/csrc/jcm_api.hip

```cpp
#include <cmath>
#include <cstdlib>
#include <cstdio>
#include <cstring>

#include <mutex>
#include <vector>

#include "ctx.h"

using namespace jcm;

namespace {
thread_local std::string g_err;
}

namespace jcm {

const char* const kJointNames[10] = {"lsho", "lelb", "lwri", "rsho", "relb", "rwri", "lhip", "rhip", "nose", "torso"};

int fail(int code, const std::string& msg) {
  g_err = msg;
  return code;
}

// ... 99 lines not shown
    t[i] = find(c, name);
    if (!t[i]) return fail(JCM_ERR_STATE, "missing parameter '" + name + "'");
    if (t[i]->n != (size_t)n) return fail(JCM_ERR_STATE, "parameter '" + name + "' has " + std::to_string(t[i]->n) + " elements, expected " + std::to_string(n));
  }
  if (!*scale) JCM_TRY(dev_alloc(c, reinterpret_cast<void**>(scale), n * sizeof(float)));
  if (!*shift) JCM_TRY(dev_alloc(c, reinterpret_cast<void**>(shift), n * sizeof(float)));
  HIP_TRY(bn_fold(t[0]->d, t[1]->d, t[2]->d, t[3]->d, kBnEps, *scale, *shift, n, c->stream));
  return JCM_OK;
}

int check(jcm_handle h, bool need_final) {
  if (!h) return fail(JCM_ERR_ARG, "null handle");
  if (need_final && !h->finalized) return fail(JCM_ERR_STATE, "jcm_finalize has not been called");
  return JCM_OK;
}

const ConvLayer* conv_of(jcm_ctx* c, const std::string& scope) {
  auto it = c->convs.find(scope);
  return it == c->convs.end() ? nullptr : &it->second;
}

static int launch_conv_layer(jcm_ctx* c, const ConvLayer* L, const void* wp, const void* x, int B, int H, int W, void* out, bool act_bf16,
                             bool out_f32, int in_planar, int out_planar) {
  ConvArgs a{};
  a.x = x; a.wp = wp; a.bias = L->bias; a.scale = L->scale; a.shift = L->shift; a.out = out;
  a.B = B; a.H = H; a.W = W; a.Cin = L->cin; a.Cout = L->cout; a.relu_bn = L->has_bn ? 1 : 0;
  a.in_planar = in_planar; a.out_planar = out_planar;
  a.hpool = c->conv_hpool;
  c->conv_hpool = 0;
  if ((in_planar || out_planar) && !act_bf16) return fail(JCM_ERR_ARG, "planar activations exist on the bf16 path only");
  if (a.hpool && !act_bf16) return fail(JCM_ERR_STATE, "half pool requested on an fp32 layer");
  if (act_bf16) {
    a.CoutP = L->coutp_bf16;
    if (a.hpool && (out_f32 || L->thin_bf16 || L->ks != 5 || conv_igemm_bf16_bn(L->cout, L->ks) != 128 || !conv5_strip_bf16_supported(a, L->ks)))
      return fail(JCM_ERR_STATE, "half pool requested for a layer that does not run on conv5_strip_bf16_kernel");
    if (L->thin_bf16 && out_f32 && L->wp_kxfold && conv_kxfold_bf16_supported(a, L->ks)) {
      a.wp = L->wp_kxfold;
      HIP_TRY(conv_kxfold_bf16(a, c->stream));
    } else if (L->thin_bf16 && out_f32) {
      HIP_TRY(conv_thin_bf16(a, c->stream));
    }
    else HIP_TRY(conv_igemm_bf16(a, L->ks, out_f32, c->stream));
  } else {
    a.CoutP = L->coutp;
    const bool use_split = L->wp_split && (L->thin ? c->f32_conv == 2 : conv_split_supported(L->ks, L->cin, L->coutp_split, B, H, W, c->split_min_wgs));
    if (use_split) {
      HIP_TRY(pow2_scale_of(static_cast<const float*>(x), (size_t)B * H * W * L->cin, c->act_scale, c->scale_scratch, c->stream));
      a.in_scale = c->act_scale;
      a.w_scale = L->wscale;
    }
    if (L->thin && L->wp_split && c->f32_conv == 2) {
      a.wp = L->wp_split;
      a.CoutP = 16;
      HIP_TRY(conv_thin_split16(a, c->stream));
    } else if (L->thin) {
      HIP_TRY(conv_thin_f32(a, c->stream));
    } else if (use_split) {
      a.wp = L->wp_split;
      a.CoutP = L->coutp_split;
      HIP_TRY(conv_split_f32(a, L->ks, 2, c->stream));
    } else {
      HIP_TRY(conv_igemm_f32(a, L->ks, c->stream));
    }
  }
  return JCM_OK;
}

static int pool_get(jcm_ctx* c, hipEvent_t* e) {
  if (!c->event_pool.empty()) {
    *e = c->event_pool.back();
    c->event_pool.pop_back();
    return JCM_OK;
  }
  HIP_TRY(hipEventCreate(e));
  return JCM_OK;
}
int prof_begin(jcm_ctx* c, hipEvent_t* e0, hipEvent_t* e1) {
  *e0 = *e1 = nullptr;
  if (!c->profile) return JCM_OK;
  JCM_TRY(pool_get(c, e0));
  if (int r = pool_get(c, e1); r != JCM_OK) { c->event_pool.push_back(*e0); *e0 = nullptr; return r; }
  hipError_t e = hipEventRecord(*e0, c->stream);
  if (e != hipSuccess) {
    prof_end(c, "", *e0, *e1, false);
    *e0 = *e1 = nullptr;
    return fail(JCM_ERR_HIP, std::string("hipEventRecord: ") + hipGetErrorString(e));
  }
  return JCM_OK;
}
void prof_end(jcm_ctx* c, const std::string& scope, hipEvent_t e0, hipEvent_t e1, bool ok) {
  if (!e0) return;
  if (ok && hipEventRecord(e1, c->stream) == hipSuccess) {
    c->prof[scope].emplace_back(e0, e1);
  } else {
    c->event_pool.push_back(e0);
    c->event_pool.push_back(e1);
  }
}
void prof_release_all(jcm_ctx* c, bool destroy) {
  for (auto& kv : c->prof)
    for (auto& ev : kv.second) { c->event_pool.push_back(ev.first); c->event_pool.push_back(ev.second); }
  c->prof.clear();
  if (destroy) {
    for (hipEvent_t e : c->event_pool) (void)hipEventDestroy(e);
    c->event_pool.clear();
  }
}

bool takes_fft(jcm_ctx* c, const ConvLayer* L, int B, int H, int W) {
  if (!c->conv9_fft || c->f32_conv != 0 || (c->train && c->precision != JCM_PRECISION_F32) || (L->ks != 9 && L->ks != 5) || L->cin == 3 || !L->w_raw) return false;
  if (c->precision == JCM_PRECISION_BF16 && (L->ks != 9 || L->thin_bf16 || L->cout % 8)) return false;
  ConvArgs a{};
  a.B = B; a.H = H; a.W = W; a.Cin = L->cin; a.Cout = L->cout;
  return conv_fft_supported(a, L->ks);
}
bool fft_spectra_valid(jcm_ctx* c, const std::string& scope, int H, int W, int circ) {
  auto it = c->fft_w.find(scope + (circ ? "@win" : "@") + std::to_string(H) + "x" + std::to_string(W));
  return it != c->fft_w.end() && it->second.valid;
}
int fft_new_words(jcm_ctx* c, int n, float** w) {
  if (n < 1) return fail(JCM_ERR_ARG, "fft_new_words: n < 1");
  for (;;) {
    if (c->fft_block_i < (int)c->fft_blocks.size()) {
      jcm_ctx::WordBlock& b = c->fft_blocks[c->fft_block_i];
      if (c->fft_word_i + n <= b.cap) {
        *w = b.p + c->fft_word_i;
        c->fft_word_i += n;
        return JCM_OK;
      }
      ++c->fft_block_i;
      c->fft_word_i = 0;
      continue;
    }
    jcm_ctx::WordBlock b;
    b.cap = n > jcm_ctx::kFftWords ? n : jcm_ctx::kFftWords;
    HIP_TRY(hipMalloc(reinterpret_cast<void**>(&b.p), (size_t)b.cap * sizeof(float)));
    if (hipError_t e = hipMemsetAsync(b.p, 0, (size_t)b.cap * sizeof(float), c->stream); e != hipSuccess) {
      (void)hipFree(b.p);
      return fail(JCM_ERR_HIP, std::string("hipMemsetAsync: ") + hipGetErrorString(e));
    }
    c->fft_blocks.push_back(b);
  }
}
int run_conv_fft(jcm_ctx* c, const ConvLayer* L, const std::string& scope, const void* x, int B, int H, int W, void* out, int in_layout, int out_layout, int circ) {
  ConvArgs a{};
  a.x = x; a.bias = L->bias; a.scale = L->scale; a.shift = L->shift; a.out = out;
  a.B = B; a.H = H; a.W = W; a.Cin = L->cin; a.Cout = L->cout; a.CoutP = L->cout; a.relu_bn = L->has_bn ? 1 : 0;
  a.circ = circ;
  a.rows_mfma = c->fft_rows_mfma;
  const size_t mark = c->arena_off;
  const int np = fft_np(c);
  a.tiles = c->fft_tiles && c->fft_next_pool && !c->fft_t_in && !c->fft_xs && !c->fft_merge && !c->fft_win_map && !circ && in_layout == 0 &&
            np == 4 && conv_fft_tiles_supported(a, L->ks, c->fft_next_ks) ? 1 : 0;
  const int wH = a.tiles ? H / 2 : H, wW = a.tiles ? W / 2 : W;
  void* work = arena_alloc<char>(c, conv_fft_workspace_bytes(a, L->ks, np));
  c->arena_off = mark;
  if (c->dry) { c->fft_t_in = nullptr; c->fft_t_next = nullptr; c->fft_merge = nullptr; c->fft_xs = nullptr; c->fft_xs_ready = false; c->fft_tmax_in = nullptr; c->fft_next_pool = 0; c->fft_next_ks = 0; c->fft_next_merge = nullptr; c->fft_t_in_16 = false; c->fft_win_map = nullptr; c->fft_win_scatter = false; return JCM_OK; }
  const std::string key = scope + (circ ? "@win" : "@") + std::to_string(wH) + "x" + std::to_string(wW);
  if (!c->fft_w.count(key)) {
    static const size_t cap = [] { const char* e = std::getenv("JCM_FFT_CACHE_GB"); return (size_t)(e ? std::atoi(e) : 64) << 30; }();
    const size_t need = conv_fft_weight_bytes(wH, wW, L->ks, L->cin, L->cout, np, circ);
    size_t held = 0;
    for (auto& kv : c->fft_w) held += kv.second.bytes;
    if (held + need > cap && !c->fft_w.empty()) {
      HIP_TRY(hipStreamSynchronize(c->stream));
      for (auto& kv : c->fft_w) (void)hipFree(kv.second.p);
      c->fft_w.clear();
    }
  }
  jcm_ctx::FftW& fw = c->fft_w[key];
  if (!fw.p) {
    const size_t wb = (conv_fft_weight_bytes(wH, wW, L->ks, L->cin, L->cout, np, circ) + 255) & ~size_t(255);
    fw.bytes = wb + 256;
    if (hipMalloc(&fw.p, fw.bytes) == hipSuccess) {
      fw.wscale = reinterpret_cast<float*>(static_cast<char*>(fw.p) + wb);
    } else {
      const size_t mb = fw.bytes >> 20;
      c->fft_w.erase(key);
      return fail(JCM_ERR_HIP, "out of device memory for the filter spectra of '" + scope + "' (" + std::to_string(mb) + " MB); jcm_set_option(\"conv9_fft\", 0) selects the direct kernels");
    }
  }
  if (!fw.valid) {
    const float* bound_from = nullptr;
    if (np >= 4 && scope.compare(0, 6, "dgrad:") == 0) {
      auto it = c->fft_w.find(key.substr(6));
      if (it != c->fft_w.end() && it->second.valid && it->second.wscale) bound_from = it->second.wscale;
    }
    HIP_TRY(conv_fft_pack_weights(L->w_raw, fw.p, wH, wW, L->ks, L->cin, L->cout, np, c->precision == JCM_PRECISION_BF16, c->stream, fw.wscale, circ, bound_from));
    fw.valid = true;
  }
  a.wp = fw.p;
  hipEvent_t e0 = nullptr, e1 = nullptr, g0 = nullptr, g1 = nullptr;
  JCM_TRY(prof_begin(c, &e0, &e1));
  if (c->profile && (pool_get(c, &g0) != JCM_OK || pool_get(c, &g1) != JCM_OK)) { g0 = g1 = nullptr; }
  const void* t_in = c->fft_t_in;
  void* t_next = c->fft_t_next;
  const FftMerge* mg = static_cast<const FftMerge*>(c->fft_merge);
  void* xs = c->fft_xs;
  const bool xs_ready = c->fft_xs_ready;
  FftNext nx;
  nx.pool = c->fft_next_pool; nx.ks_next = c->fft_next_ks; nx.merge = static_cast<const FftMerge*>(c->fft_next_merge);
  c->fft_next_pool = 0; c->fft_next_ks = 0; c->fft_next_merge = nullptr;
  const bool t_in_16 = c->fft_t_in_16;
  c->fft_t_in_16 = false;
  if (c->fft_win_map) {
    a.win_map = c->fft_win_map; a.win_B = c->fft_win_B; a.win_H = c->fft_win_H; a.win_W = c->fft_win_W; a.win_TY = c->fft_win_TY; a.win_TX = c->fft_win_TX;
    c->fft_win_map = nullptr;
  }
  if (c->fft_win_scatter) {
    a.wout_H = c->fft_win_H; a.wout_W = c->fft_win_W; a.wout_TY = c->fft_win_TY; a.wout_TX = c->fft_win_TX;
    c->fft_win_scatter = false;
  }
  Fp16Scale sc;
  if (np >= 4) {
    sc.tmax = c->fft_tmax_in;
    if ((t_in || xs_ready) && !sc.tmax) return fail(JCM_ERR_STATE, "conv_fft '" + scope + "': a handed-over tensor without its scale word");
    if (!sc.tmax) JCM_TRY(fft_new_words(c, a.tiles ? 4 * B : B, &sc.tmax));
    if (t_next) JCM_TRY(fft_new_words(c, B, &sc.tmax_next));
    sc.winv = fw.wscale + 1;
    sc.common = c->train ? 1 : 0;
    sc.t16 = (np == 5 && c->fft_t16 && in_layout != 0 && out_layout != 0 && !xs && (!t_in || t_in_16) && (!t_next || (nx.merge && !t_in))) ? 1 : 0;
  }
  c->fft_t_in = nullptr; c->fft_t_next = nullptr; c->fft_merge = nullptr; c->fft_xs = nullptr; c->fft_xs_ready = false;
  c->fft_tmax_in = sc.tmax_next;
  c->fft_last_tmax = sc.tmax;
  const hipError_t e = conv_fft_f32(a, L->ks, np, in_layout, out_layout, work, t_in, t_next, mg, g0, g1, c->stream, xs, xs_ready, np >= 4 ? &sc : nullptr, &nx);
  if (g0 && g1 && e == hipSuccess) c->prof[scope + "/gemm"].emplace_back(g0, g1);
  else { if (g0) c->event_pool.push_back(g0); if (g1) c->event_pool.push_back(g1); }
  prof_end(c, scope, e0, e1, e == hipSuccess);
  if (e != hipSuccess) return fail(JCM_ERR_HIP, std::string("conv_fft_f32: ") + hipGetErrorString(e));
  return JCM_OK;
}

int run_conv_layer(jcm_ctx* c, const ConvLayer* L, const std::string& scope, int stride, const void* x, int B, int H, int W, int sub,
                   void* out, bool act_bf16, bool out_f32, int in_planar, int out_planar) {
  if (stride == 2) {
    if (c->dry) return JCM_OK;
    if (!(L->ks == 5 && L->cin == 3 && L->has_bn))
      return fail(JCM_ERR_ARG, "stride-2 kernel exists for 5x5, Cin=3, BN layers only (" + scope + ")");
    HIP_TRY(conv1_5x5s2(static_cast<const float*>(x), L->w_raw, L->bias, L->scale, L->shift, out, act_bf16, B, H, W, sub,
                        L->cout, c->stream));
    return JCM_OK;
  }
  if (stride == 1 && takes_fft(c, L, B, H, W))
    return run_conv_fft(c, L, scope, x, B, H, W, out, act_bf16 ? (in_planar ? 2 : 1) : 0, (act_bf16 && !out_f32) ? (out_planar ? 2 : 1) : 0);
  if (c->dry) return JCM_OK;
  const void* wp = act_bf16 ? L->wp_bf16 : static_cast<const void*>(L->wp);
  if (stride != 1 || !wp) return fail(JCM_ERR_ARG, "no kernel for layer '" + scope + "' with stride " + std::to_string(stride));
  if (!act_bf16 && L->wp_stale) {
    HIP_TRY(pack_weights_f32(L->w_raw, L->wp, L->ks, L->cin, L->cout, L->coutp, c->stream));
    L->wp_stale = false;
  }
  hipEvent_t e0 = nullptr, e1 = nullptr;
  JCM_TRY(prof_begin(c, &e0, &e1));
  const int r = launch_conv_layer(c, L, wp, x, B, H, W, out, act_bf16, out_f32, in_planar, out_planar);
  prof_end(c, scope, e0, e1, r == JCM_OK);
  return r;
}

}

namespace jcm {

static int weight_scale(jcm_ctx* c, const Tensor& w, float** wscale) {
  if (!c->scale_scratch) {
    JCM_TRY(dev_alloc(c, reinterpret_cast<void**>(&c->scale_scratch), 1024 * sizeof(float)));
    JCM_TRY(dev_alloc(c, reinterpret_cast<void**>(&c->act_scale), 2 * sizeof(float)));
  }
  if (!*wscale) JCM_TRY(dev_alloc(c, reinterpret_cast<void**>(wscale), 2 * sizeof(float)));
  HIP_TRY(pow2_scale_of(w.d, w.n, *wscale, c->scale_scratch, c->stream));
  return JCM_OK;
}

int refresh_derived(jcm_ctx* c, bool first) {
  for (auto& kv : c->fft_w) kv.second.valid = false;
  for (auto& kv : c->params) {
    const std::string& name = kv.first;
    const std::string suffix = "/weights";
    if (name.size() <= suffix.size() || name.compare(name.size() - suffix.size(), suffix.size(), suffix) != 0) continue;
    const Tensor& w = kv.second;
    if (w.shape.size() != 4 || w.shape[0] != w.shape[1]) return fail(JCM_ERR_ARG, "'" + name + "' must be [k,k,Cin,Cout]");
    const std::string scope = name.substr(0, name.size() - suffix.size());
    ConvLayer L;
    if (!first) {
      auto it = c->convs.find(scope);
      if (it == c->convs.end()) return fail(JCM_ERR_STATE, "conv layer '" + scope + "' appeared after jcm_finalize");
      L = it->second;
    }
    L.ks = (int)w.shape[0]; L.cin = (int)w.shape[2]; L.cout = (int)w.shape[3];
    L.w_raw = w.d;
    const Tensor* b = find(c, scope + "/biases");
    if (!b || b->n != (size_t)L.cout) return fail(JCM_ERR_STATE, "missing or mis-sized '" + scope + "/biases'");
    L.bias = b->d;
    L.has_bn = find(c, scope + "/BatchNorm/gamma") != nullptr;
    if (L.has_bn) JCM_TRY(fold_bn(c, scope, L.cout, &L.scale, &L.shift));
    if ((L.ks == 5 || L.ks == 9) && L.cin % 16 == 0 && c->precision == JCM_PRECISION_F32) {
      L.thin = L.ks == 9 && L.cout <= 12;
      const int bn = L.thin ? 16 : conv_igemm_bn(L.cout);
      L.coutp = (L.cout + bn - 1) / bn * bn;
      const size_t n = (size_t)L.ks * L.ks * L.cin * L.coutp;
      if (!L.wp) JCM_TRY(dev_alloc(c, reinterpret_cast<void**>(&L.wp), n * sizeof(float)));
      if (first) HIP_TRY(pack_weights_f32(w.d, L.wp, L.ks, L.cin, L.cout, L.coutp, c->stream));
      else L.wp_stale = true;
    }
    if (c->precision == JCM_PRECISION_F32 && c->f32_conv == 2 && (L.ks == 9 || L.ks == 5) && L.cin % 16 == 0 && L.cout % 128 == 0) {
      const int ns = 2;
      L.coutp_split = L.cout;
      if (!L.wp_split) JCM_TRY(dev_alloc(c, &L.wp_split, conv_split_weight_bytes(L.ks, L.cin, L.coutp_split, ns)));
      JCM_TRY(weight_scale(c, w, &L.wscale));
      HIP_TRY(pack_weights_split(w.d, L.wp_split, L.ks, L.cin, L.cout, L.coutp_split, ns, c->stream, L.wscale));
    }
    if (c->precision == JCM_PRECISION_F32 && c->f32_conv == 2 && L.ks == 9 && L.cout <= 16 && L.cin % 32 == 0) {
      L.coutp_split = 16;
      if (!L.wp_split) JCM_TRY(dev_alloc(c, &L.wp_split, conv_split_weight_bytes(L.ks, L.cin, 16, 2)));
      JCM_TRY(weight_scale(c, w, &L.wscale));
      HIP_TRY(pack_weights_split(w.d, L.wp_split, L.ks, L.cin, L.cout, 16, 2, c->stream, L.wscale));
    }
    if (L.ks == 5 && L.cin == 3 && L.cout == 64 && L.has_bn && c->precision == JCM_PRECISION_F32) {
      if (!L.wq1_f32) JCM_TRY(dev_alloc(c, reinterpret_cast<void**>(&L.wq1_f32), 5 * 16 * 64 * sizeof(float)));
      HIP_TRY(pack_conv1_f32(w.d, L.wq1_f32, c->stream));
      if (!L.wq1_split) JCM_TRY(dev_alloc(c, &L.wq1_split, conv1_split_weight_bytes()));
      HIP_TRY(pack_conv1_split(w.d, L.wq1_split, c->stream));
    }
    if (L.ks == 5 && L.cin == 3 && L.cout == 64 && L.has_bn && c->precision == JCM_PRECISION_BF16) {
      if (!L.wq1_bf16) JCM_TRY(dev_alloc(c, &L.wq1_bf16, 5 * 2 * 64 * 16));
      HIP_TRY(pack_conv1_bf16(w.d, L.wq1_bf16, c->stream));
    }
    if ((L.ks == 5 || L.ks == 9) && c->precision == JCM_PRECISION_BF16 && L.cin != 3) {
      if (L.cin % 32 != 0) return fail(JCM_ERR_ARG, "bf16 path needs Cin % 32 == 0 ('" + scope + "' has " + std::to_string(L.cin) + ")");
      L.thin_bf16 = L.ks == 9 && L.cout <= 16 && !L.has_bn;
      const int bn = L.thin_bf16 ? 16 : conv_igemm_bf16_bn(L.cout, L.ks);
      L.coutp_bf16 = (L.cout + bn - 1) / bn * bn;
      const size_t n = (size_t)L.ks * L.ks * L.cin * L.coutp_bf16;
      if (!L.wp_bf16) JCM_TRY(dev_alloc(c, &L.wp_bf16, n * 2));
      HIP_TRY(pack_weights_bf16(w.d, L.wp_bf16, L.ks, L.cin, L.cout, L.coutp_bf16, c->stream));
      if (L.thin_bf16 && L.cout == 9) {
        if (!L.wp_kxfold) JCM_TRY(dev_alloc(c, &L.wp_kxfold, conv_kxfold_weight_bytes(L.cin)));
        HIP_TRY(pack_weights_kxfold(w.d, L.wp_kxfold, L.cin, c->stream));
      }
    }
    c->convs[scope] = L;
// ... 176 lines not shown
    const int hp = pl23 && c->bf16_hpool && w2 % 2 == 0 && !(sk & 6) ? 1 : 0;
    c->conv_hpool = hp;
    if (!(sk & 4)) JCM_TRY(run_conv(c, "conv2_" + res, 1, p1, B, h2, w2, 1, c2, bf, false, 0, pl23));
    c->conv_hpool = 0;
    void* p2 = t23 ? nullptr : act((size_t)B * h3 * w3 * L2->cout);
    if (!c->dry && !(sk & 2) && !t23) {
      if (hp) HIP_TRY(vpool_2x1_bf16(c2, p2, B * (L2->cout / 8), h2, w2 / 2, 8, c->stream));
      else if (pl23) HIP_TRY(max_pool_2x2(c2, p2, bf, B * (L2->cout / 8), h2, w2, 8, c->stream));
      else HIP_TRY(max_pool_2x2(c2, p2, bf, B, h2, w2, L2->cout, c->stream));
    }
    const ConvLayer* L4r = conv_of(c, "conv4_" + res);
    if (!L4r) return fail(JCM_ERR_STATE, "part-detector parameters incomplete (conv4_" + res + ")");
    const int in4 = planar && L3->cout % 8 == 0 && takes_strip(L4r, B, h3, w3) && !takes_fft(c, L4r, B, h3, w3) ? 1 : 0;
    void* t34 = (sk & 24) ? nullptr : offer_handover(c, L3, L4r, B, h3, w3);
    void* c3 = t34 ? nullptr : act((size_t)B * h3 * w3 * L3->cout);
    c->fft_t_in = t23;
    if (!(sk & 8)) JCM_TRY(run_conv(c, "conv3_" + res, 1, p2, B, h3, w3, 1, c3, bf, false, pl23, in4));
    c->fft_t_in = t34;
    if (r == 0 && fuse45) { c->fft_t_next = t45; c->fft_next_merge = &mg; }
    if (!(sk & 16)) JCM_TRY(run_conv(c, "conv4_" + res, 1, c3, B, h3, w3, 1, x4[r], bf, false, in4, planar45));
    c->arena_off = mark;
  }
  const bool fuse_merge = !fuse45 && takes_fft(c, L5, B, hh, ww) && !planar45;
  void* merged = fuse45 ? nullptr : fuse_merge ? x4[0] : act((size_t)B * hh * ww * L4->cout);
  if (!c->dry && !fuse45 && !fuse_merge && !(c->debug_skip & 32)) {
    if (planar45) HIP_TRY(upsample_merge3_planar(x4[0], x4[1], h4[1], w4[1], x4[2], h4[2], w4[2], merged, B, hh, ww, L4->cout, c->stream));
    else HIP_TRY(upsample_merge3(x4[0], x4[1], h4[1], w4[1], x4[2], h4[2], w4[2], merged, bf, B, hh, ww, L4->cout, c->stream));
  }
  const int sk = c->debug_skip;
  void* t56 = (sk & 96) ? nullptr : offer_handover(c, L5, conv_of(c, "conv6"), B, hh, ww);
  void* c5 = t56 ? nullptr : act((size_t)B * hh * ww * L5->cout);
  if (fuse_merge && !(sk & 32)) c->fft_merge = &mg;
  if (fuse45) { c->fft_t_in = t45; c->fft_t_in_16 = h16; }
  if (!(sk & 32)) JCM_TRY(run_conv(c, "conv5", 1, merged, B, hh, ww, 1, c5, bf, false, planar45, planar));
  c->fft_t_in = t56;
  if (!(sk & 64)) JCM_TRY(run_conv(c, "conv6", 1, c5, B, hh, ww, 1, logits, bf, true, planar, 0));
  return JCM_OK;
}

int sm_forward_impl(jcm_ctx* c, const float* hm, int Ca, const float* extra, int B, float* logits, int extra_ld = 0) {
  if (extra_ld <= 0) extra_ld = kC - Ca;
  if (!c->has_sm) return fail(JCM_ERR_STATE, "spatial-model parameters (bn_sm, energy_*, bias_*) were not set");
  const int P = c->K * (kC - 1);
  if (c->sm_algo == 1) {
    float* lik = arena_alloc<float>(c, (size_t)B * kC * kHmH * 96);
    float* cpre = arena_alloc<float>(c, (size_t)B * P * kCH * kCW);
    if (c->dry) return JCM_OK;
    HIP_TRY(sm_likelihood(hm, Ca, extra, c->bn_sm_scale, c->bn_sm_shift, lik, B, kC, c->stream, extra_ld));
    HIP_TRY(sm_pair_conv(c->sp_energy, lik, c->cond, cpre, B, P, kC, c->stream));
    HIP_TRY(sm_finish(lik, cpre, c->sp_bias, logits, B, c->K, kC, c->stream));
    return JCM_OK;
  }
  if (c->sm_algo == 3) {
    float2* lhat_t = arena_alloc<float2>(c, (size_t)B * kC * kSpec);
    if (c->dry) return JCM_OK;
    void* scr = nullptr;
    unsigned epoch = 0;
    JCM_TRY(sm_scratch_next(c, &scr, &epoch));
    HIP_TRY(sm_fused_forward(hm, Ca, extra, extra_ld, c->bn_sm_scale, c->bn_sm_shift, c->prior_spec_t, c->cond, c->sp_bias, lhat_t, logits, B, c->K, kC,
                             c->stream, nullptr, scr, epoch));
    return JCM_OK;
  }
  return fail(JCM_ERR_STATE, "sm_algo must be 3 (transforms in LDS) or 1 (direct)");
}

}

extern "C" {

int jcm_abi_version(void) { return 1; }

const char* jcm_last_error(void) { return g_err.c_str(); }

int jcm_create(int device, void* stream, jcm_handle* out) {
  if (!out) return fail(JCM_ERR_ARG, "null out pointer");
  int n = 0;
  HIP_TRY(hipGetDeviceCount(&n));
  if (device < 0 || device >= n) return fail(JCM_ERR_ARG, "device " + std::to_string(device) + " out of range (" + std::to_string(n) + " visible)");
  hipDeviceProp_t prop;
  HIP_TRY(hipGetDeviceProperties(&prop, device));
  if (std::strncmp(prop.gcnArchName, "gfx950", 6) != 0)
    return fail(JCM_ERR_HIP, std::string("libjcm is built for gfx950 (MI355X) only; device reports ") + prop.gcnArchName);
  jcm_ctx* c = new jcm_ctx();
  c->device = device;
  c->stream = static_cast<hipStream_t>(stream);
  *out = c;
  return JCM_OK;
}

int jcm_destroy(jcm_handle h) {
  if (!h) return JCM_OK;
  DeviceGuard g(h->device);
  (void)hipStreamSynchronize(h->stream);
  prof_release_all(h, true);
  if (h->train) train_destroy(h);
  for (auto& kv : h->params) (void)hipFree(kv.second.d);
  for (void* p : h->owned) (void)hipFree(p);
  for (auto& kv : h->fft_w) (void)hipFree(kv.second.p);
  for (auto& b : h->fft_blocks) (void)hipFree(b.p);
  if (h->arena) (void)hipFree(h->arena);
  delete h;
  return JCM_OK;
}

int jcm_set_option(jcm_handle h, const char* key, int64_t value) {
  JCM_TRY(check(h, false));
  const std::string k = key ? key : "";
  if (k == "profile") {
    if (value != 0 && !h->profile) {
      DeviceGuard g(h->device);
      (void)hipStreamSynchronize(h->stream);
      prof_release_all(h, false);
    }
    h->profile = value != 0;
    return JCM_OK;
  }
  if (k == "micro_batch") {
    if (value < 0) return fail(JCM_ERR_ARG, "micro_batch must be >= 0 (0 = default: 256 bf16 / 64 fp32)");
    h->micro_batch = (int)value;
    return JCM_OK;
  }
  if (k == "debug_skip") {
    h->debug_skip = (int)value;
    return JCM_OK;
  }
  if (k == "call_order") {
    h->call_order = value != 0;
    return JCM_OK;
  }
  if (k == "conv9_fft") {
    h->conv9_fft = value != 0;
    return JCM_OK;
  }
  if (k == "fft_single") {
    if ((value != 0) != (h->fft_single != 0)) {
      HIP_TRY(hipStreamSynchronize(h->stream));
      for (auto& kv : h->fft_w) (void)hipFree(kv.second.p);
      h->fft_w.clear();
    }
    h->fft_single = value != 0;
    return JCM_OK;
  }
  if (k == "fft_windows") {
    h->fft_win = value != 0;
    return JCM_OK;
  }
  if (k == "fft_fuse") {
    if (value < 0 || value > 3) return fail(JCM_ERR_ARG, "fft_fuse must be 0..3 (bit 0: pool hand-over, bit 1: merge hand-over)");
    h->fft_fuse = (int)value;
    return JCM_OK;
  }
  if (k == "fft_tiles") {
    h->fft_tiles = value != 0;
    return JCM_OK;
  }
  if (k == "bf16_hpool") {
    h->bf16_hpool = value != 0;
    return JCM_OK;
  }
  if (k == "fft_rows_mfma") {
    h->fft_rows_mfma = value != 0;
    return JCM_OK;
  }
  if (k == "fft_t16") {
    h->fft_t16 = value != 0;
    return JCM_OK;
  }
  if (k == "sm_chunk") {
    if (value < 1) return fail(JCM_ERR_ARG, "sm_chunk must be >= 1");
    h->sm_chunk = (int)value;
    return JCM_OK;
  }
  if (k == "split_min_wgs") {
    if (value < 0) return fail(JCM_ERR_ARG, "split_min_wgs must be >= 0");
    h->split_min_wgs = (int)value;
    return JCM_OK;
  }
  if (k == "sm_algo") {
    if (value != 1 && value != 3) return fail(JCM_ERR_ARG, "sm_algo must be 3 (every transform in LDS, default) or 1 (direct sliding-window kernel); the rocFFT routes 0 and 2 were removed in round 5");
    h->sm_algo = (int)value;
    return JCM_OK;
  }
  if (h->finalized) return fail(JCM_ERR_STATE, "options must be set before jcm_finalize");
  if (k == "precision") {
    if (value != JCM_PRECISION_F32 && value != JCM_PRECISION_BF16) return fail(JCM_ERR_ARG, "precision must be 0 (f32) or 1 (bf16)");
    h->precision = (int)value;
  } else if (k == "f32_conv") {
    if (value != 0 && value != 2) return fail(JCM_ERR_ARG, "f32_conv must be 0 (default) or 2 (fp16x3 direct split kernels); 1 (bf16x6) was retired in round 5");
    h->f32_conv = (int)value;
  } else if (k == "n_joints") {
    if (value < 1 || value > 9) return fail(JCM_ERR_ARG, "n_joints must be in [1,9]");
    h->K = (int)value;
  } else {
    return fail(JCM_ERR_ARG, "unknown option '" + k + "'");
  }
  return JCM_OK;
}

int jcm_set_tensor(jcm_handle h, const char* name, const float* data, const int64_t* shape, int ndim) {
  JCM_TRY(check(h, false));
  if (h->finalized) return fail(JCM_ERR_STATE, "parameters must be set before jcm_finalize");
  if (!name || !data || !shape || ndim < 1 || ndim > 4) return fail(JCM_ERR_ARG, "bad set_tensor arguments");
  DeviceGuard g(h->device);
  CallOrder order(h);
  size_t n = 1;
  for (int i = 0; i < ndim; ++i) {
    if (shape[i] <= 0) return fail(JCM_ERR_ARG, std::string("non-positive dimension in '") + name + "'");
    n *= (size_t)shape[i];
  }
  Tensor& t = h->params[name];
  if (t.d) { (void)hipFree(t.d); h->param_bytes -= t.n * sizeof(float); }
  t.shape.assign(shape, shape + ndim);
  t.n = n;
  t.d = nullptr;
  HIP_TRY(hipMalloc(reinterpret_cast<void**>(&t.d), n * sizeof(float)));
  h->param_bytes += n * sizeof(float);
  HIP_TRY(hipMemcpyAsync(t.d, data, n * sizeof(float), hipMemcpyDefault, h->stream));
  order.release();
  HIP_TRY(hipStreamSynchronize(h->stream));
  return JCM_OK;
}

int jcm_finalize(jcm_handle h) {
  JCM_TRY(check(h, false));
  if (h->finalized) return fail(JCM_ERR_STATE, "already finalized");
  DeviceGuard g(h->device);
  CallOrder order(h);
  JCM_TRY(refresh_derived(h, true));
  h->finalized = true;
  return JCM_OK;
}

int jcm_conv_layer(jcm_handle h, const char* scope, int stride, int last_layer, const float* x, int B, int H, int W, float* out) {
  JCM_TRY(check(h, true));
  if (!scope || !x || !out || B < 1 || H < 1 || W < 1) return fail(JCM_ERR_ARG, "bad conv_layer arguments");
  DeviceGuard g(h->device);
  CallOrder order(h);
  const ConvLayer* L = conv_of(h, scope);
  if (!L) return fail(JCM_ERR_STATE, std::string("no conv layer '") + scope + "'");
  if ((last_layer != 0) == L->has_bn)
    return fail(JCM_ERR_ARG, std::string("last_layer flag disagrees with the BatchNorm parameters stored for '") + scope + "'");
  if (h->precision == JCM_PRECISION_F32)
    return with_arena(h, [&] { return run_conv(h, scope, stride, x, B, H, W, 1, out, false, false); });
  if (stride != 1) return fail(JCM_ERR_ARG, "bf16 handles run the stride-2 first layer fused with its pool inside jcm_pd_forward only");
  jcm_ctx* c = h;
  return with_arena(c, [&] {
    const size_t nin = (size_t)B * H * W * L->cin, nout = (size_t)B * H * W * L->cout;
    void* xb = arena_alloc<char>(c, nin * 2);
    void* ob = last_layer ? nullptr : static_cast<void*>(arena_alloc<char>(c, nout * 2));
    if (!c->dry) HIP_TRY(cast_pad_bf16(x, L->cin, xb, L->cin, (size_t)B * H * W, c->stream));
    JCM_TRY(run_conv(c, scope, 1, xb, B, H, W, 1, last_layer ? static_cast<void*>(out) : ob, true, last_layer != 0));
    if (!c->dry && !last_layer) HIP_TRY(cast_bf16_f32(ob, out, nout, c->stream));
    return (int)JCM_OK;
  });
}

int jcm_conv_layer_merged(jcm_handle h, const char* scope, const float* x1, const float* x2, int H2, int W2, const float* x3, int H3, int W3, int B, int H, int W,
                          float* out) {
  JCM_TRY(check(h, true));
  if (!scope || !x1 || !x2 || !x3 || !out || B < 1 || H < 1 || W < 1 || H2 < 1 || W2 < 1 || H3 < 1 || W3 < 1) return fail(JCM_ERR_ARG, "bad conv_layer_merged arguments");
  DeviceGuard g(h->device);
  CallOrder order(h);
  jcm_ctx* c = h;
  const ConvLayer* L = conv_of(c, scope);
  if (!L) return fail(JCM_ERR_STATE, std::string("no conv layer '") + scope + "'");
  if (!L->has_bn) return fail(JCM_ERR_ARG, "conv_layer_merged: a layer with BatchNorm parameters is expected (conv5)");
  const bool bf = c->precision != JCM_PRECISION_F32;
  if (bf && L->cin % 8) return fail(JCM_ERR_ARG, "conv_layer_merged: Cin % 8 != 0 on a bf16 handle");
  return with_arena(c, [&] {
    const size_t n1 = (size_t)B * H * W * L->cin, n2 = (size_t)B * H2 * W2 * L->cin, n3 = (size_t)B * H3 * W3 * L->cin, nout = (size_t)B * H * W * L->cout;
    const void *a1 = x1, *a2 = x2, *a3 = x3;
    void* ob = out;
    if (bf) {
      void* b1 = arena_alloc<char>(c, n1 * 2);
      void* b2 = arena_alloc<char>(c, n2 * 2);
      void* b3 = arena_alloc<char>(c, n3 * 2);
      ob = arena_alloc<char>(c, nout * 2);
      if (!c->dry) {
        HIP_TRY(cast_pad_bf16(x1, L->cin, b1, L->cin, (size_t)B * H * W, c->stream));
        HIP_TRY(cast_pad_bf16(x2, L->cin, b2, L->cin, (size_t)B * H2 * W2, c->stream));
        HIP_TRY(cast_pad_bf16(x3, L->cin, b3, L->cin, (size_t)B * H3 * W3, c->stream));
      }
      a1 = b1; a2 = b2; a3 = b3;
    }
    FftMerge mg{a2, H2, W2, a3, H3, W3};
    const void* in = a1;
    if (takes_fft(c, L, B, H, W)) {
      c->fft_merge = &mg;
    } else {
      void* merged = arena_alloc<char>(c, n1 * (bf ? 2 : 4));
      if (!c->dry) HIP_TRY(upsample_merge3(a1, a2, H2, W2, a3, H3, W3, merged, bf, B, H, W, L->cin, c->stream));
      in = merged;
    }
    JCM_TRY(run_conv(c, scope, 1, in, B, H, W, 1, ob, bf, false));
    if (bf && !c->dry) HIP_TRY(cast_bf16_f32(ob, out, nout, c->stream));
    return (int)JCM_OK;
  });
}

int jcm_max_pool(jcm_handle h, const float* x, int B, int H, int W, int C, float* out) {
  JCM_TRY(check(h, false));
  if (!x || !out || B < 1 || H < 1 || W < 1 || C < 1 || C % 4) return fail(JCM_ERR_ARG, "bad max_pool arguments (C must be a multiple of 4)");
  DeviceGuard g(h->device);
  CallOrder order(h);
  HIP_TRY(max_pool_2x2(x, out, false, B, H, W, C, h->stream));
  return JCM_OK;
// ... 270 lines not shown
```

### joint-cnn-mrf_amd/csrc/kernels.h

```cpp
#pragma once
#include <hip/hip_runtime.h>
#include <stdint.h>

#include <atomic>

namespace jcm {

struct LdsAttr {
  std::atomic<uint64_t> done{0};
  hipError_t ensure(const void* fn, int bytes) {
    int dev = 0;
    hipError_t e = hipGetDevice(&dev);
    if (e != hipSuccess) return e;
    const uint64_t bit = 1ull << (dev & 63);
    if (done.load(std::memory_order_acquire) & bit) return hipSuccess;
    e = hipFuncSetAttribute(fn, hipFuncAttributeMaxDynamicSharedMemorySize, bytes);
    if (e == hipSuccess) done.fetch_or(bit, std::memory_order_release);
    return e;
  }
};

struct ConvArgs {
  const void* x;
  const void* wp;
  const float* bias;
  const float* scale;
  const float* shift;
  void* out;
  int B, H, W, Cin, Cout, CoutP;
  int relu_bn;
  const float* in_scale = nullptr;
  const float* w_scale = nullptr;
  int in_planar = 0, out_planar = 0;
  int circ = 0;
  const void* win_map = nullptr;
  int win_B = 0, win_H = 0, win_W = 0, win_TY = 0, win_TX = 0, win_valid_only = 0;
  int wout_H = 0, wout_W = 0, wout_TY = 0, wout_TX = 0;
  int tiles = 0;
  int rows_mfma = 0;
  int hpool = 0;
};
int conv_igemm_bn(int Cout);
hipError_t conv_igemm_f32(const ConvArgs& a, int ks, hipStream_t st);
hipError_t pack_weights_f32(const float* w_hwio, float* wp, int ks, int Cin, int Cout, int CoutP, hipStream_t st);

bool conv_split_supported(int ks, int Cin, int CoutP, int B, int H, int W, int min_wgs);
size_t conv_split_weight_bytes(int ks, int Cin, int CoutP, int ns);
hipError_t pack_weights_split(const float* w_hwio, void* wp, int ks, int Cin, int Cout, int CoutP, int ns, hipStream_t st,
                              const float* w_scale = nullptr);
hipError_t conv_split_f32(const ConvArgs& a, int ks, int ns, hipStream_t st);

hipError_t conv_thin_split16(const ConvArgs& a, hipStream_t st);

hipError_t conv_thin_f32(const ConvArgs& a, hipStream_t st);

hipError_t conv_thin_bf16(const ConvArgs& a, hipStream_t st);

struct Fp16Scale {
  float* tmax = nullptr;
  float* tmax_next = nullptr;
  const float* winv = nullptr;
  float hf = 0.f;
  int nb = 0;
  int common = 0;
  int t16 = 0;
  float* t16_fwd = nullptr;
  float* t16_inv = nullptr;
  int t16_cb = 64;
};
bool conv_fft_supported(const ConvArgs& a, int ks);
size_t conv_fft_weight_bytes(int H, int W, int ks, int Cin, int Cout, int np, int circ = 0);
hipError_t conv_fft_pack_weights(const float* w_hwio, void* wf, int H, int W, int ks, int Cin, int Cout, int np, bool round_bf16, hipStream_t st,
                                 float* wscale = nullptr, int circ = 0,
                                 const float* bound_from = nullptr);
size_t conv_fft_workspace_bytes(const ConvArgs& a, int ks, int np);
struct FftMerge { const void* x2; int H2, W2; const void* x3; int H3, W3; };
struct FftNext { int pool = 0; int ks_next = 0; const FftMerge* merge = nullptr; };
hipError_t conv_fft_f32(const ConvArgs& a, int ks, int np, int in_layout, int out_layout, void* work, const void* t_in, void* t_next, const FftMerge* merge,
                        hipEvent_t g0, hipEvent_t g1, hipStream_t st, void* xs = nullptr, bool xs_ready = false, const Fp16Scale* sc = nullptr, const FftNext* nx = nullptr);
bool conv_fft_win_gather_supported(int win, int Cin);
bool conv_fft_win_scatter_supported(int win, int Cout);
bool conv_fft_pool_fusable(const ConvArgs& a, int ks, int ks_next);
bool conv_fft_tiles_supported(const ConvArgs& a, int ks, int ks_next);
size_t conv_fft_pool_handover_bytes(const ConvArgs& a, int ks_next);
bool conv_fft_merge_fusable(const ConvArgs& a, int ks, int ks_next, const FftMerge& m, bool h16 = false);
size_t conv_fft_xs_bytes(const ConvArgs& a, int ks, int np);
hipError_t conv_fft_spectra(const ConvArgs& a, int ks, int np, void* work, void* xs, hipStream_t st, float* tmax = nullptr, int common = 0);
bool conv_fft_geometry(int H, int W, int ks, int B, int Cout, int np, int* NY, int* NX, int* MT, int circ = 0);

size_t wgrad_fft_scratch_bytes(int NY, int NX, int Cin, int Cout);
hipError_t wgrad_fft(const void* xs, const void* zs, void* scratch, const float* w, float lmbd, float* dw, int ks, int NY, int NX, int B, int MTx, int MTz, int Cin,
                     int ldz, int Cout, hipStream_t st, int np = 3, const float* tmax_x = nullptr, const float* tmax_z = nullptr, int H = 0);
hipError_t pad_channels_f32(const float* in, int ldi, float* out, int ldo, size_t N, hipStream_t st);
hipError_t window_gather_f32(const float* map, float* win, int B, int H, int W, int C, int WS, int TY, int TX, int valid_only, hipStream_t st);
hipError_t window_scatter_f32(const float* val, float* map, int B, int H, int W, int C, int WS, int TY, int TX, hipStream_t st);
bool conv_fft_fusable(const ConvArgs& a, int ks, int ks_next);
size_t conv_fft_handover_bytes(const ConvArgs& a, int ks);

int cgemm_split_mtile(int np, int B, int Cout);
int cgemm_split_ntile(int np, int Cout);
int cgemm_split_parts(int np);
size_t cgemm_split_w_bytes(int np, int F, int Cin, int Cout);
float cgemm_split_y16_shift(int Cin);
hipError_t cgemm_split(const void* xs, const void* ws, void* y, int np, int F, int B, int Cin, int Cout, int ldy, hipStream_t st, float y16_shift = 0.f);

bool conv5_strip_bf16_supported(const ConvArgs& a, int ks);
hipError_t conv5_strip_bf16(const ConvArgs& a, hipStream_t st);

bool conv_kxfold_bf16_supported(const ConvArgs& a, int ks);
size_t conv_kxfold_weight_bytes(int Cin);
hipError_t pack_weights_kxfold(const float* w_hwio, void* wp, int Cin, hipStream_t st);
hipError_t conv_kxfold_bf16(const ConvArgs& a, hipStream_t st);

int conv_igemm_bf16_bn(int Cout, int ks);
hipError_t conv_igemm_bf16(const ConvArgs& a, int ks, bool out_f32, hipStream_t st);
hipError_t pack_weights_bf16(const float* w_hwio, void* wp, int ks, int Cin, int Cout, int CoutP, hipStream_t st);

bool conv_strip_bf16_supported(const ConvArgs& a, int ks);
hipError_t conv_strip_bf16(const ConvArgs& a, hipStream_t st);

hipError_t conv1_5x5s2(const float* x, const float* w, const float* bias, const float* scale, const float* shift,
                       void* out, bool out_bf16, int B, int H0, int W0, int sub, int Cout, hipStream_t st);

hipError_t pack_conv1_bf16(const float* w_hwio, void* wq, hipStream_t st);
hipError_t conv1_mfma_pool(const float* x, const void* wq, const float* bias, const float* scale, const float* shift,
                           void* out, int B, int H0, int W0, int sub, hipStream_t st);

hipError_t pack_conv1_f32(const float* w_hwio, float* wq, hipStream_t st);
size_t conv1_split_weight_bytes();
hipError_t pack_conv1_split(const float* w_hwio, void* wq, hipStream_t st);
hipError_t conv1_mfma_pool_split(const float* x, const void* wq, const float* bias, const float* scale, const float* shift, float* out,
                                 int B, int H0, int W0, int sub, hipStream_t st);
hipError_t conv1_mfma_pool_f32(const float* x, const float* wq, const float* bias, const float* scale, const float* shift, float* out,
                               int B, int H0, int W0, int sub, hipStream_t st);

hipError_t max_pool_2x2(const void* x, void* out, bool bf16, int B, int H, int W, int C, hipStream_t st);
hipError_t vpool_2x1_bf16(const void* x, void* out, int B, int H, int W, int C, hipStream_t st);
hipError_t resize_bilinear(const float* x, float* out, int B, int H, int W, int C, int OH, int OW, hipStream_t st);
hipError_t upsample_merge3(const void* x1, const void* x2, int H2, int W2, const void* x3, int H3, int W3,
                           void* out, bool bf16, int B, int H, int W, int C, hipStream_t st);
hipError_t upsample_merge3_planar(const void* x1, const void* x2, int H2, int W2, const void* x3, int H3, int W3,
                                  void* out, int B, int H, int W, int C, hipStream_t st);
hipError_t spatial_softmax(const float* in, float* out, int B, int HW, int K, hipStream_t st);
hipError_t argmax_coords(const float* hm, int32_t* coords, int B, int HW, int WW, int K, hipStream_t st);
hipError_t softmax_argmax(const float* logits, float* prob, int32_t* coords, int B, int HW, int WW, int K, hipStream_t st);
hipError_t bn_fold(const float* gamma, const float* beta, const float* mean, const float* var, float eps, float* scale, float* shift,
                   int n, hipStream_t st);

hipError_t sm_softplus5(const float* in, float* out, int64_t n, hipStream_t st);
hipError_t sm_softplus5_multi(const float* const* in, float* out, int P, int64_t n, hipStream_t st);
hipError_t sm_likelihood(const float* hm, int Ca, const float* extra, const float* bn_scale, const float* bn_shift, float* lik,
                         int B, int C, hipStream_t st, int extra_ld = 0);
hipError_t sm_pair_conv(const float* priors, const float* maps, const int* cond, float* cpre,
                        int B, int P, int C, hipStream_t st);
hipError_t sm_finish(const float* lik, const float* cpre, const float* spbias, float* logits,
                     int B, int K, int C, hipStream_t st);
hipError_t sm_resize_only(const float* cpre, float* out, int B, hipStream_t st);

hipError_t sm_pad_frame(const float* hm, int Ca, const float* extra, const float* sc, const float* sh, float* frame, int B, int C,
                        hipStream_t st, int extra_ld = 0);
hipError_t sm_spec_mul(const float2* lhat, const float2* phat, const int* cond, float2* spec, int B, int C, int P, hipStream_t st);
hipError_t sm_resize_frame(const float* cfull, float* out, int B, hipStream_t st);
hipError_t sm_fused_forward(const float* hm, int Ca, const float* extra, int extra_ld, const float* sc, const float* sh, const float2* phat_t,
                            const int* cond, const float* spbias, float2* lhat_t, float* logits, int B, int K, int C, hipStream_t st,
                            float* tsave, void* scratch, unsigned epoch);
size_t sm_fused_scratch_bytes();
hipError_t sm_fused_spectra(const float* hm, int Ca, const float* extra, int extra_ld, const float* sc, const float* sh, float2* lhat_t, int B, int C,
                            hipStream_t st);
hipError_t sm_lds_fwd_frames(const float* frames, float2* spec_t, int n, hipStream_t st);
hipError_t sm_lds_fwd_dframes(const float* G, const float* T, float2* dhat_t, int nb, int K, int P, hipStream_t st);
hipError_t sm_lds_inv_frames(const float2* spec_t, float* frames, int n, int r0, int nrows, float scale, hipStream_t st);

hipError_t window_resize(const float* src, int H, int W, int C, const int* windows_dev, int NW, float2* mm_scratch,
                         int OH, int OW, float* out, hipStream_t st);
hipError_t group_mean(const float* in, float* out, int n, int G, size_t M, hipStream_t st);

size_t augment_scratch_doubles(int B);
hipError_t augment_train(const float* x, const float* y, const float* params, int B, int H, int W, int hh, int hw, double* scratch,
                         float* x_out, float* y_out, hipStream_t st);

size_t train_reduce_scratch_doubles(int C);
hipError_t bn_batch_stats(const void* x, bool bf16, size_t N, int C, float eps, float decay, float* mean, float* rstd, float* mov_mean,
                          float* mov_var, double* scratch, hipStream_t st);
hipError_t bn_apply(const void* r, const float* mean, const float* rstd, const float* gamma, const float* beta, void* y, bool bf16, size_t N,
                    int C, hipStream_t st);
hipError_t bn_bwd_reduce(const void* dy, float dy_scale, const void* r, bool bf16, const float* mean, const float* rstd, size_t N, int C,
                         float* sums, float* dgamma, float* dbeta, double* scratch, hipStream_t st);
hipError_t bn_bwd_apply(const void* dy, float dy_scale, const void* r, bool bf16, const float* mean, const float* rstd, const float* gamma,
                        const float* sums, size_t N, int C, int relu, void* dz, hipStream_t st);
hipError_t col_sum(const void* x, bool bf16, size_t N, int C, float* out, double* scratch, hipStream_t st);
bool bn_apply_pool(const void* r, const float* mean, const float* rstd, const float* gamma, const float* beta, void* y, void* p, bool bf16, int B, int H, int W, int C,
                   hipStream_t st);
bool bn_bwd_pooled(const void* dp, const void* y, const void* r, bool bf16, const float* mean, const float* rstd, const float* gamma, int B, int H, int W, int C, float* sums,
                   float* dgamma, float* dbeta, void* dz, float* colsum, double* scratch, hipStream_t st, hipError_t* err);
hipError_t bn_bwd_apply_colsum(const void* dy, float dy_scale, const void* r, bool bf16, const float* mean, const float* rstd, const float* gamma, const float* sums, size_t N,
                               int C, int relu, void* dz, float* colsum, double* scratch, hipStream_t st);
hipError_t max_pool_bwd(const void* x, const void* dy, void* dx, bool bf16, int B, int H, int W, int C, hipStream_t st);
hipError_t cast_pad_bf16(const float* in, int ldi, void* out, int ldo, size_t N, hipStream_t st);
hipError_t cast_bf16_f32(const void* in, float* out, size_t n, hipStream_t st);
hipError_t resize_bilinear_bwd(const void* dy, void* dx, bool bf16, int B, int h, int w, int H, int W, int C, float scale, hipStream_t st);
hipError_t softmax_ce(const float* logits, const float* target, int B, int HW, int K, int Kt, float gscale, float* loss, float* dz,
                      int ldz, int accumulate, hipStream_t st);
hipError_t softmax_bwd(const float* p, const float* g, int B, int HW, int K, int ldg, float* dz, int ldz, hipStream_t st);
hipError_t loss_means_accumulate(const float* ce, int n, float scale, float* out, bool first, hipStream_t st);
hipError_t sum_squares(const float* x, size_t n, double* out, int accumulate, double* scratch, hipStream_t st);
hipError_t sum_squares_chunks(float* const* w, const int64_t* start, const int* len, const int* flag, int nchunks, double* out, double* scratch, hipStream_t st);
hipError_t adam_update(float* w, const float* g, float* m, float* v, size_t n, const double* sumsq, float clip, float lr_t, float b1,
                       float b2, float eps, hipStream_t st);
hipError_t momentum_update(float* w, const float* g, float* acc, size_t n, const double* sumsq, float clip, float lr, float mom,
                           hipStream_t st);
hipError_t scale_copy(const float* a, float s, float* out, size_t n, hipStream_t st);
hipError_t optimizer_chunks(float* const* wptr, const int64_t* cstart, const int64_t* coff, const int* clen, int nchunks, const float* g,
                            float* m, float* v, const double* sumsq, float clip, float lr_t, float b1, float b2, float eps, int momentum_mode,
                            hipStream_t st);

int wgrad_splits(int ks, int Cin, int Cout, int B, int H);
hipError_t wgrad_f32(const float* x, const float* dz, float* partial, int splits, int ks, int B, int H, int W, int Cin, int Cout, int ldz,
                     hipStream_t st);
hipError_t wgrad_reduce(const float* partial, int splits, size_t n, const float* w, float lmbd, float* dw, hipStream_t st, const float* out_scale = nullptr);
int wgrad_conv1_blocks(void);
hipError_t wgrad_reduce_wide(const float* partial, int splits, size_t n, const float* w, float lmbd, float* dw, hipStream_t st);
hipError_t wgrad_conv1(const float* x, const void* dz, bool dz_bf16, float* partial, int B, int H0, int W0, int sub, int Cout, hipStream_t st);
hipError_t split_parts16(const float* x, void* out_f16_2n, size_t n, const float* scale, hipStream_t st);
hipError_t pow2_scale_of(const float* x, size_t n, float* scale, float* scratch, hipStream_t st);
hipError_t wgrad_split16(const void* xp, const void* zp, float* partial, int splits, int ks, int B, int H, int W, int Cin, int Cout, int ldz,
                         hipStream_t st);
bool wgrad_split_supported(int ks, int Cin, int ldz);
hipError_t wgrad_bf16(const void* x, const void* dz, float* partial, int splits, int ks, int B, int H, int W, int Cin, int Cout, int ldz,
                      hipStream_t st);
hipError_t flip_transpose_weights(const float* w_hwio, float* wd, int ks, int Cin, int Cout, int CoP, hipStream_t st);

hipError_t bn_fold_stats(const float* mean, const float* rstd, const float* gamma, const float* beta, float* sc, float* sh, int n,
                         hipStream_t st);
hipError_t sm_concat_target(const float* prob, const float* y, float* out, size_t N, int K, int C, hipStream_t st);
hipError_t sm_bwd_dbias(const float* G, const float* T, float* dspb, int nb, int K, int P, int accumulate, hipStream_t st);
hipError_t sm_bwd_spec_da(const float2* Dhat, const float2* Lhat, const int* cond, float2* dA, int nb, int C, int P, int accumulate,
// ... 9 lines not shown
```

### joint-cnn-mrf_amd/engine.py

```python
import ctypes

import numpy as np
import torch

from . import _lib


def _hm_size(n):
    for _ in range(3):
        n = (n + 1) // 2
    return n


class Engine:

    def __init__(self, device=0, precision='fp32', n_joints=9, stream=None, f32_conv=None, split_min_wgs=None, micro_batch=None, conv9_fft=None, call_order=None, fft_single=None, fft_t16=None, fft_fuse=None, fft_tiles=None):
        if not torch.cuda.is_available():
            raise RuntimeError('joint-cnn-mrf_amd needs an MI355X (gfx950) GPU; torch.cuda.is_available() is False '
                               'and there is no CPU path')
        self._lib = _lib.load()
        self.device = torch.device('cuda', device if isinstance(device, int) else torch.device(device).index or 0)
        self.n_joints = int(n_joints)
        self.precision = precision
        self._stream = stream if stream is not None else torch.cuda.current_stream(self.device)
        h = ctypes.c_void_p()
        _lib.check(self._lib.jcm_create(self.device.index, ctypes.c_void_p(self._stream.cuda_stream), ctypes.byref(h)),
                   'jcm_create')
        self._h = h
        self._finalized = False
        prec = {'fp32': _lib.JCM_PRECISION_F32, 'f32': _lib.JCM_PRECISION_F32, 'bf16': _lib.JCM_PRECISION_BF16}[precision]
        _lib.check(self._lib.jcm_set_option(self._h, b'precision', prec), 'jcm_set_option(precision)')
        _lib.check(self._lib.jcm_set_option(self._h, b'n_joints', self.n_joints), 'jcm_set_option(n_joints)')
        if f32_conv is not None:
            if f32_conv not in ('exact', 'split16'):
                raise ValueError("f32_conv must be 'exact' or 'split16' (the bf16x6 arm 'split' was retired in round 5)")
            _lib.check(self._lib.jcm_set_option(self._h, b'f32_conv', {'exact': 0, 'split16': 2}[f32_conv]), 'jcm_set_option(f32_conv)')
        if micro_batch is not None:
            self.set_micro_batch(micro_batch)
        if conv9_fft is not None:
            self.set_conv9_fft(conv9_fft)
        if fft_single is not None:
            self.set_option('fft_single', int(bool(fft_single)))
        if fft_t16 is not None:
            self.set_option('fft_t16', int(bool(fft_t16)))
        if fft_fuse is not None:
            self.set_option('fft_fuse', int(fft_fuse))
        if fft_tiles is not None:
            self.set_option('fft_tiles', int(bool(fft_tiles)))
        if call_order is not None:
            self.set_option('call_order', int(bool(call_order)))
        if split_min_wgs is not None:
            _lib.check(self._lib.jcm_set_option(self._h, b'split_min_wgs', int(split_min_wgs)), 'jcm_set_option(split_min_wgs)')

    def close(self):
        if getattr(self, '_h', None) is not None and self._h.value:
            self._lib.jcm_destroy(self._h)
            self._h = ctypes.c_void_p()

    def __del__(self):
        try:
            self.close()
        except Exception:
            pass

    def set_tensor(self, name, value):
        if isinstance(value, torch.Tensor):
            t = value.detach().to(torch.float32).contiguous()
            ptr, shape, keep = t.data_ptr(), tuple(t.shape), t
        else:
            a = np.ascontiguousarray(value, dtype=np.float32)
            ptr, shape, keep = a.ctypes.data, a.shape, a
        if len(shape) == 0:
            raise ValueError('scalar parameter %r' % name)
        arr = (ctypes.c_int64 * len(shape))(*shape)
        _lib.check(self._lib.jcm_set_tensor(self._h, name.encode(), ctypes.c_void_p(ptr), arr, len(shape)),
                   'jcm_set_tensor(%s)' % name)
        del keep

    def load_params(self, params, finalize=True):
        for name, value in params.items():
            self.set_tensor(name, value)
        if finalize:
            self.finalize()
        return self

    def update_tensor(self, name, value, refresh=True):
        a = np.ascontiguousarray(value, dtype=np.float32)
        _lib.check(self._lib.jcm_update_tensor(self._h, name.encode(), ctypes.c_void_p(a.ctypes.data), a.size, int(bool(refresh))),
                   'jcm_update_tensor(%s)' % name)

    def finalize(self):
        _lib.check(self._lib.jcm_finalize(self._h), 'jcm_finalize')
        self._finalized = True

    def _chk(self, t, ndim, name, dtype=torch.float32):
        if not isinstance(t, torch.Tensor):
            raise TypeError('%s must be a torch tensor' % name)
        if t.device != self.device:
            raise ValueError('%s is on %s, engine is on %s' % (name, t.device, self.device))
        if t.dtype != dtype:
            raise TypeError('%s must be %s, got %s' % (name, dtype, t.dtype))
        if t.dim() != ndim:
            raise ValueError('%s must have %d dims (NHWC), got shape %s' % (name, ndim, tuple(t.shape)))
        if not t.is_contiguous():
            raise ValueError('%s must be contiguous (NHWC)' % name)
        return t

    def _new(self, *shape, dtype=torch.float32):
        return torch.empty(shape, dtype=dtype, device=self.device)

    @staticmethod
    def _p(t):
        return ctypes.c_void_p(t.data_ptr()) if t is not None else ctypes.c_void_p(0)

    def conv_layer(self, x, name, stride, last_layer=False, n_out=None):
        self._chk(x, 4, 'x')
        B, H, W, _ = x.shape
        if n_out is None:
            raise ValueError('n_out is required to size the output')
        out = self._new(B, -(-H // stride), -(-W // stride), n_out)
        _lib.check(self._lib.jcm_conv_layer(self._h, name.encode(), stride, int(bool(last_layer)), self._p(x), B, H, W,
                                            self._p(out)), 'jcm_conv_layer(%s)' % name)
        return out

    def conv_layer_merged(self, x1, x2, x3, name, n_out):
        for t, nm in ((x1, 'x1'), (x2, 'x2'), (x3, 'x3')):
            self._chk(t, 4, nm)
        B, H, W, C = x1.shape
        if x2.shape[0] != B or x3.shape[0] != B or x2.shape[3] != C or x3.shape[3] != C:
            raise ValueError('x1, x2, x3 must share batch and channel counts')
        out = self._new(B, H, W, n_out)
        _lib.check(self._lib.jcm_conv_layer_merged(self._h, name.encode(), self._p(x1), self._p(x2), x2.shape[1], x2.shape[2], self._p(x3), x3.shape[1], x3.shape[2],
                                                   B, H, W, self._p(out)), 'jcm_conv_layer_merged(%s)' % name)
        return out

    def max_pool(self, x):
        self._chk(x, 4, 'x')
        B, H, W, C = x.shape
        out = self._new(B, (H + 1) // 2, (W + 1) // 2, C)
        _lib.check(self._lib.jcm_max_pool(self._h, self._p(x), B, H, W, C, self._p(out)), 'jcm_max_pool')
        return out

    def resize_bilinear(self, x, oh, ow):
        self._chk(x, 4, 'x')
        B, H, W, C = x.shape
        out = self._new(B, oh, ow, C)
        _lib.check(self._lib.jcm_resize_bilinear(self._h, self._p(x), B, H, W, C, oh, ow, self._p(out)), 'jcm_resize_bilinear')
        return out

    def model(self, x):
        self._chk(x, 4, 'x')
        B, H, W, C = x.shape
        if C != 3:
            raise ValueError('x must be [B,H,W,3], got %s' % (tuple(x.shape),))
        out = self._new(B, _hm_size(H), _hm_size(W), self.n_joints)
        _lib.check(self._lib.jcm_pd_forward(self._h, self._p(x), B, H, W, self._p(out)), 'jcm_pd_forward')
        return out

    def spatial_softmax(self, hm):
        self._chk(hm, 4, 'hm')
        B, H, W, K = hm.shape
        out = torch.empty_like(hm)
        _lib.check(self._lib.jcm_spatial_softmax(self._h, self._p(hm), B, H * W, K, self._p(out)), 'jcm_spatial_softmax')
        return out

    def conv_mrf(self, A, Bm):
        self._chk(A, 4, 'A')
        self._chk(Bm, 4, 'B')
        if tuple(A.shape) != (1, 120, 180, 1) or tuple(Bm.shape[1:]) != (60, 90, 1):
            raise ValueError('conv_mrf expects A [1,120,180,1] and B [b,60,90,1]; got %s, %s' % (tuple(A.shape), tuple(Bm.shape)))
        out = torch.empty_like(Bm)
        _lib.check(self._lib.jcm_conv_mrf(self._h, self._p(A), self._p(Bm), Bm.shape[0], self._p(out)), 'jcm_conv_mrf')
        return out

    def spatial_model(self, heat_map):
        self._chk(heat_map, 4, 'heat_map')
        B = heat_map.shape[0]
        if tuple(heat_map.shape[1:]) != (60, 90, self.n_joints + 1):
            raise ValueError('spatial_model expects [B,60,90,%d], got %s' % (self.n_joints + 1, tuple(heat_map.shape)))
        out = self._new(B, 60, 90, self.n_joints)
        _lib.check(self._lib.jcm_sm_forward(self._h, self._p(heat_map), B, self._p(out)), 'jcm_sm_forward')
        return out

    def argmax_coords(self, hm):
        self._chk(hm, 4, 'hm')
        B, H, W, K = hm.shape
        out = self._new(B, 2, K, dtype=torch.int32)
        _lib.check(self._lib.jcm_argmax_coords(self._h, self._p(hm), B, H, W, K, self._p(out)), 'jcm_argmax_coords')
        return out

    def softmax_argmax(self, logits, want_prob=True):
        self._chk(logits, 4, 'logits')
        B, H, W, K = logits.shape
        prob = torch.empty_like(logits) if want_prob else None
        coords = self._new(B, 2, K, dtype=torch.int32)
        _lib.check(self._lib.jcm_softmax_argmax(self._h, self._p(logits), B, H, W, K, self._p(prob), self._p(coords)), 'jcm_softmax_argmax')
        return prob, coords

    def forward(self, x, torso=None, use_sm=True, want_prob=True):
        self._chk(x, 4, 'x')
        B, H, W, C = x.shape
# ... 154 lines not shown
```

Measured before the change: 7180 images/sec.

## Split 60-row FFT convolutions into two overlapping y-tiles with 40-point transforms

Adds a y-tiling mode for 9x9 FFT convolutions on 60x90 maps with large channel counts. Each map is split into two 30-row tiles with 4-row halos and transformed with a 40-point column FFT instead of the full padded height, which doubles the effective batch but shrinks the frequency grid. Weight spectra are cached separately as circular 40x96 spectra, and the inverse uses a new 40-point register kernel. The intent is to cut spectral work and the channel GEMM size per image, at the cost of halo overhead and an extra weight-spectrum set.

```diff
diff --git a/joint-cnn-mrf_amd/csrc/conv_fft.hip b/joint-cnn-mrf_amd/csrc/conv_fft.hip
--- a/joint-cnn-mrf_amd/csrc/conv_fft.hip
+++ b/joint-cnn-mrf_amd/csrc/conv_fft.hip
@@ -171,6 +171,10 @@
 }
 static bool fft_tiles_on() {
   static const bool on = [] { const char* e = std::getenv("JCM_FFT_TILES"); return !e || std::atoi(e) != 0; }();
+  return on;
+}
+static bool fft_ytiles_on() {
+  static const bool on = [] { const char* e = std::getenv("JCM_FFT_YTILES"); return !e || std::atoi(e) != 0; }();
   return on;
 }
 static int padn(int c, int n) { return (c + n - 1) / n * n; }
@@ -283,11 +287,23 @@
   t.tiles = 0;
   return t;
 }
+ConvArgs ytile_view(const ConvArgs& a) {
+  ConvArgs t = a;
+  t.B = 2 * a.B; t.H = a.H / 2;
+  t.ytiles = 0;
+  return t;
+}
+}
+bool conv_fft_ytiles_supported(const ConvArgs& a, int ks, int np) {
+  Sizes s;
+  return fft_reg_on() && fft_ytiles_on() && np == 4 && ks == 9 && !a.circ && !a.win_map && !a.tiles && a.wout_TX == 0 && a.B >= 1 && a.H == 60 && a.W == 90 &&
+         a.H / 2 + 8 <= kFftYtileNY && (size_t)a.Cin * a.Cout >= (size_t)256 * 512 && a.Cin % CB == 0 && a.Cout % CB == 0 && sizes_of(a.H, a.W, ks, &s) && tw_offset(kFftYtileNY) >= 0;
 }
 size_t conv_fft_workspace_bytes(const ConvArgs& a, int ks, int np) {
   Sizes s;
   if (!(a.tiles ? sizes_of(a.H / 2, a.W / 2, ks, &s) : sizes_of(a.H, a.W, ks, &s, a.circ))) return 0;
-  const Plan3 p = a.tiles ? plan_of(tile_view(a, s), s, np) : plan_of(a, s, np);
+  if (a.ytiles) s.NY = kFftYtileNY;
+  const Plan3 p = a.tiles ? plan_of(tile_view(a, s), s, np) : a.ytiles ? plan_of(ytile_view(a), s, np) : plan_of(a, s, np);
   return align256(p.t_bytes) + align256(p.xs_bytes) + align256(p.yf_bytes) + align256(p.sc_fwd_bytes) + align256(p.sc_inv_bytes);
 }
 bool conv_fft_fusable(const ConvArgs& a, int ks, int ks_next) {
@@ -361,11 +377,14 @@
   if (!conv_fft_supported(a0, ks) || !sizes_of(a0.H, a0.W, ks, &s, a0.circ) || (out_layout == 2 && a0.Cout % 8) || (np != 2 && np != 4 && np != 5) || (np == 5 && a0.Cin % 32)) return hipErrorInvalidValue;
   if (a0.circ && (t_in || t_next || merge || in_layout != 0 || out_layout != 0)) return hipErrorInvalidValue;
   if (nx && (nx->pool || nx->merge) && (!t_next || (nx->pool && nx->merge))) return hipErrorInvalidValue;
+  const bool yt = a0.ytiles != 0;
+  if (yt && (!conv_fft_ytiles_supported(a0, ks, np) || in_layout != 0 || out_layout != 0 || xs || xs_ready || !scp || scp->common || scp->t16)) return hipErrorInvalidValue;
+  if (yt) s.NY = kFftYtileNY;
   Fp16Scale sc;
   if (np >= 4) {
     if (!scp || !scp->tmax || !scp->winv || (t_next && !scp->tmax_next)) return hipErrorInvalidValue;
     sc = *scp;
-    sc.hf = (float)a0.H;
+    sc.hf = yt ? (float)(a0.H / 2 + 8) : (float)a0.H;
     sc.nb = a0.B;
   }
   const bool h16 = sc.t16 && ((t_next && nx && nx->merge && !t_in) || (t_in && !t_next));
@@ -376,7 +395,8 @@
   ConvArgs a = a0;
   a.CoutP = pad64(a.Cout);
   const int opad = (ks - 1) / 2 + (a0.circ ? 4 : 0);
-  const Plan3 p = plan_of(a, s, np);
+  const ConvArgs av = yt ? ytile_view(a) : a;
+  const Plan3 p = plan_of(av, s, np);
   char* wk = static_cast<char*>(work);
   cf* T = reinterpret_cast<cf*>(wk);
   void* Xs = xs ? xs : wk + align256(p.t_bytes);
@@ -404,16 +424,18 @@
       if (a.win_map) { if (!cfft_rows_fwd_win_reg(s.NX, a, T, sc.tmax, st)) return hipErrorInvalidValue; }
       else if (!(fft_reg && cfft_rows_fwd_reg(s.NX, a, in_layout, T, sc.tmax, st, sc.t16_fwd))) cfft_rows_fwd(s.NX, a, in_layout, T, twx, sc.tmax, st, sc.t16_fwd);
     }
-    if (hipError_t ce = cfft_cols_fwd(s.NY, a, np, Tin, Xs, twy, p.NXH, p.MT, sc, st); ce != hipSuccess) return ce;
+    if (hipError_t ce = cfft_cols_fwd(s.NY, a, np, Tin, Xs, twy, p.NXH, p.MT, sc, st, yt ? a.H / 2 : 0); ce != hipSuccess) return ce;
   }
   if (hipError_t e = hipGetLastError(); e != hipSuccess) return e;
   if (g0 && hipEventRecord(g0, st) != hipSuccess) return hipErrorUnknown;
   const float yshift = sc.t16 ? cgemm_split_y16_shift(a.Cin) : 0.f, yinv = yshift != 0.f ? 1.0f / yshift : 0.f;
-  if (hipError_t e = cgemm_split(Xs, a.wp, Yf, np, p.F, a.B, a.Cin, a.Cout, p.ldy, st, yshift); e != hipSuccess) return e;
+  if (hipError_t e = cgemm_split(Xs, a.wp, Yf, np, p.F, av.B, a.Cin, a.Cout, p.ldy, st, yshift); e != hipSuccess) return e;
   if (g1 && hipEventRecord(g1, st) != hipSuccess) return hipErrorUnknown;
   ConvArgs ai = a;
   if (a0.circ) { ai.H = a0.H - 8; ai.W = a0.W - 8; }
-  if (!(fft_reg && p.inv_cb == 64 && cfft_cols_inv_reg(s.NY, ai, Yf, T, p.NXH, p.ldy, opad, st, sc.t16_inv, yinv))) cfft_cols_inv(s.NY, ai, Yf, T, twy, p.NXH, p.ldy, opad, st, sc.t16_inv, yinv);
+  if (yt) {
+    if (!cfft_cols_inv_reg(s.NY, av, Yf, T, p.NXH, p.ldy, opad, st, nullptr, 0.f)) return hipErrorInvalidValue;
+  } else if (!(fft_reg && p.inv_cb == 64 && cfft_cols_inv_reg(s.NY, ai, Yf, T, p.NXH, p.ldy, opad, st, sc.t16_inv, yinv))) cfft_cols_inv(s.NY, ai, Yf, T, twy, p.NXH, p.ldy, opad, st, sc.t16_inv, yinv);
   if (t_next && nx && nx->pool) {
     Sizes sn;
     if (!sizes_of((a.H + 1) / 2, (a.W + 1) / 2, nx->ks_next, &sn) ||
diff --git a/joint-cnn-mrf_amd/csrc/conv_fft_cols.hip b/joint-cnn-mrf_amd/csrc/conv_fft_cols.hip
--- a/joint-cnn-mrf_amd/csrc/conv_fft_cols.hip
+++ b/joint-cnn-mrf_amd/csrc/conv_fft_cols.hip
@@ -3,12 +3,13 @@
 namespace jcm {
 namespace cfft {
 
-template <int NY, int NP, bool T16 = false>
+template <int NY, int NP, bool T16 = false, int YT = 0>
 __global__ __launch_bounds__(colfwd_threads<NY>()) void cols_fwd_split_kernel(const cf* __restrict__ T, uint4* __restrict__ Xs, const cf* __restrict__ twg, int B, int H, int KC, int MT,
                                                             int mtiles, const float* __restrict__ tmax, int common, const float* __restrict__ t16, int ntiles) {
   constexpr int IMG = colimg<NY>(), CH = IMG * 16, NTC = colfwd_threads<NY>(), NPP = NP == 5 ? 1 : 2;
   constexpr int CPV = T16 ? 4 : 2;
   constexpr int NV = NY * CH / CPV, KV = (NV + NTC - 1) / NTC, VPR = CH / CPV, VPI = 16 / CPV;
+  static_assert(YT == 0 || (YT + 8 <= NY && IMG % 2 == 0 && !T16), "a tile and its two 4-row halos inside the transform; both tiles of a map in one work group");
   extern __shared__ __attribute__((aligned(16))) char smem_cf[];
   cf* buf = reinterpret_cast<cf*>(smem_cf);
   cf* tw = buf + NY * CH;
@@ -27,10 +28,16 @@
   auto prefetch = [&](int tile) __attribute__((always_inline)) {
     int kc, kx, b0, nimg;
     coords(tile, kc, kx, b0, nimg);
-    const uint4* src = reinterpret_cast<const uint4*>(T) + (((size_t)kx * KC + kc) * B + b0) * H * VPI;
+    const uint4* src = reinterpret_cast<const uint4*>(T) + (YT ? ((size_t)kx * KC + kc) * (B >> 1) + (b0 >> 1) : ((size_t)kx * KC + kc) * B + b0) * H * VPI;
 #pragma unroll
     for (int i = 0; i < KV; ++i) {
       const int t = tid + i * NTC, y = t / VPR, v = t % VPR, img = v / VPI, cv = v % VPI;
+      if constexpr (YT > 0) {
+        const int ym = (img & 1) * YT + (y < YT + 4 ? y : y - NY);
+        const bool ok = t < NV && img < nimg && (y < YT + 4 || y >= NY - 4) && ym >= 0 && ym < H;
+        pre[i] = ok ? src[((size_t)(img >> 1) * H + ym) * VPI + cv] : make_uint4(0u, 0u, 0u, 0u);
+        continue;
+      }
       const bool ok = t < NV && y < H && img < nimg;
       pre[i] = ok ? src[((size_t)img * H + y) * VPI + cv] : make_uint4(0u, 0u, 0u, 0u);
       if constexpr (T16) psc[i] = ok ? t16[((size_t)(b0 + img) * (KC >> 2) + (kc >> 2)) * H + y] : 0.f;
@@ -55,7 +62,7 @@
       }
     }
     if constexpr (NP >= 4)
-      if (tid < IMG) xsc[tid] = tid < nimg ? fp16_scale(tmax_of(tmax, b0 + tid, B, common), (float)H) : 1.f;
+      if (tid < IMG) xsc[tid] = tid < nimg ? (YT ? fp16_scale(tmax[(b0 + tid) >> 1], (float)(YT + 8)) : fp16_scale(tmax_of(tmax, b0 + tid, B, common), (float)H)) : 1.f;
     __syncthreads();
     if (tile + (int)gridDim.x < ntiles) prefetch(tile + (int)gridDim.x);
     fft<NY, -1, CH, NTC>(buf, tw, tid);
@@ -146,19 +153,28 @@
 }
 
 
-template <int NY> static hipError_t launch_cols_fwd(const ConvArgs& a, int np, const cf* T, void* Xs, const cf* tw, int NXH, int MT, const Fp16Scale& sc, hipStream_t st) {
+template <int NY> static hipError_t launch_cols_fwd(const ConvArgs& a, int np, const cf* T, void* Xs, const cf* tw, int NXH, int MT, const Fp16Scale& sc, hipStream_t st, int ytile) {
   constexpr int IMG = colimg<NY>();
   constexpr int lds = (NY * IMG * 16 + NY) * (int)sizeof(cf);
-  const int KC = a.Cin / 16, mtiles = (a.B + MT - 1) / MT;
-  const int ntiles = NXH * KC * ((a.B + IMG - 1) / IMG);
-  static LdsAttr attr2, attr4, attr5, attr5h;
+  const int nimg = ytile ? 2 * a.B : a.B;
+  const int KC = a.Cin / 16, mtiles = (nimg + MT - 1) / MT;
+  const int ntiles = NXH * KC * ((nimg + IMG - 1) / IMG);
+  static LdsAttr attr2, attr4, attr5, attr5h, attr4y;
   const dim3 blk(colfwd_threads<NY>());
 #define COLS_FWD(KERNEL, ATTR, ...)                                                                              \
   do {                                                                                                           \
     if (hipError_t e = ATTR.ensure(reinterpret_cast<const void*>(KERNEL), lds); e != hipSuccess) return e;        \
     const dim3 grid((unsigned)persistent_grid(reinterpret_cast<const void*>(KERNEL), ntiles, (int)blk.x, lds));  \
-    hipLaunchKernelGGL(KERNEL, grid, blk, lds, st, T, static_cast<uint4*>(Xs), tw, a.B, a.H, KC, MT, mtiles, __VA_ARGS__, ntiles); \
+    hipLaunchKernelGGL(KERNEL, grid, blk, lds, st, T, static_cast<uint4*>(Xs), tw, nimg, a.H, KC, MT, mtiles, __VA_ARGS__, ntiles); \
   } while (0)
+  if (ytile) {
+    if constexpr (NY == kFftYtileNY) {
+      if (np != 4 || ytile != 30 || a.H != 60 || !sc.tmax || sc.common || sc.t16_fwd) return hipErrorInvalidValue;
+      COLS_FWD((cols_fwd_split_kernel<NY, 4, false, 30>), attr4y, sc.tmax, 0, (const float*)nullptr);
+      return hipSuccess;
+    }
+    return hipErrorInvalidValue;
+  }
   if (np == 5 && sc.t16_fwd) {
     if (!sc.tmax || (KC & 3)) return hipErrorInvalidValue;
     COLS_FWD((cols_fwd_split_kernel<NY, 5, true>), attr5h, sc.tmax, sc.common, sc.t16_fwd);
@@ -181,9 +197,9 @@
   if (t16) hipLaunchKernelGGL((cols_inv_kernel<NY, true>), grid, blk, 0, st, Yf, T, tw, a.B, a.H, NXH, a.CoutP, ldy, pad, t16, y16_inv);
   else hipLaunchKernelGGL((cols_inv_kernel<NY, false>), grid, blk, 0, st, Yf, T, tw, a.B, a.H, NXH, a.CoutP, ldy, pad, nullptr, 0.f);
 }
-hipError_t cfft_cols_fwd(int NY, const ConvArgs& a, int np, const cf* T, void* Xs, const cf* tw, int NXH, int MT, const Fp16Scale& sc, hipStream_t st) {
+hipError_t cfft_cols_fwd(int NY, const ConvArgs& a, int np, const cf* T, void* Xs, const cf* tw, int NXH, int MT, const Fp16Scale& sc, hipStream_t st, int ytile) {
   hipError_t e = hipSuccess;
-#define CALL(N) e = launch_cols_fwd<N>(a, np, T, Xs, tw, NXH, MT, sc, st)
+#define CALL(N) e = launch_cols_fwd<N>(a, np, T, Xs, tw, NXH, MT, sc, st, ytile)
   CFFT_BY_SIZE(NY, CALL)
 #undef CALL
   return e;
diff --git a/joint-cnn-mrf_amd/csrc/conv_fft_common.h b/joint-cnn-mrf_amd/csrc/conv_fft_common.h
--- a/joint-cnn-mrf_amd/csrc/conv_fft_common.h
+++ b/joint-cnn-mrf_amd/csrc/conv_fft_common.h
@@ -260,7 +260,7 @@
 
 void cfft_rows_fwd(int NX, const ConvArgs& a, int layout, cf* T, const cf* tw, float* tmax, hipStream_t st, float* t16 = nullptr);
 void cfft_rows_fwd_merge(int NX, const ConvArgs& a, const FftMerge& m, int in_layout, cf* T, const cf* tw, float* tmax, hipStream_t st, float* t16 = nullptr);
-hipError_t cfft_cols_fwd(int NY, const ConvArgs& a, int np, const cf* T, void* Xs, const cf* tw, int NXH, int MT, const Fp16Scale& sc, hipStream_t st);
+hipError_t cfft_cols_fwd(int NY, const ConvArgs& a, int np, const cf* T, void* Xs, const cf* tw, int NXH, int MT, const Fp16Scale& sc, hipStream_t st, int ytile = 0);
 void cfft_cols_inv(int NY, const ConvArgs& a, const cf* Yf, cf* T, const cf* tw, int NXH, int ldy, int pad, hipStream_t st, float* t16 = nullptr, float y16_inv = 0.f);
 void cfft_rows_inv(int NX, const ConvArgs& a, int layout, const cf* T, const cf* tw, int pad, float norm, const Fp16Scale& sc, hipStream_t st);
 bool cfft_rows_inv_reg(int NX, const ConvArgs& a, int layout, const cf* T, int pad, float norm, const Fp16Scale& sc, hipStream_t st);
diff --git a/joint-cnn-mrf_amd/csrc/conv_fft_rows_reg.hip b/joint-cnn-mrf_amd/csrc/conv_fft_rows_reg.hip
--- a/joint-cnn-mrf_amd/csrc/conv_fft_rows_reg.hip
+++ b/joint-cnn-mrf_amd/csrc/conv_fft_rows_reg.hip
@@ -241,6 +241,10 @@
   } while (0)
   switch (NY) {
     case 64: CI_LAUNCH(64); break;
+    case 40:
+      if (t16) return false;
+      hipLaunchKernelGGL((cols_inv_reg_kernel<40, false>), grid, blk, 0, st, Yf, static_cast<void*>(T), a.B, a.H, NXH, a.CoutP, ldy, pad, nullptr, 0.f);
+      break;
     case 36: CI_LAUNCH(36); break;
     case 32: CI_LAUNCH(32); break;
     case 20: CI_LAUNCH(20); break;
diff --git a/joint-cnn-mrf_amd/csrc/ctx.h b/joint-cnn-mrf_amd/csrc/ctx.h
--- a/joint-cnn-mrf_amd/csrc/ctx.h
+++ b/joint-cnn-mrf_amd/csrc/ctx.h
@@ -101,6 +101,7 @@
   bool fft_xs_ready = false;
   void* sm_scratch = nullptr;
   unsigned sm_epoch = 0;
+  int fft_ytiles = 1;
   int fft_tiles = 1;
   int fft_fuse = 3;
   int bf16_hpool = 1;
diff --git a/joint-cnn-mrf_amd/csrc/fft_reg.h b/joint-cnn-mrf_amd/csrc/fft_reg.h
--- a/joint-cnn-mrf_amd/csrc/fft_reg.h
+++ b/joint-cnn-mrf_amd/csrc/fft_reg.h
@@ -60,6 +60,7 @@
 template <> struct RPlan<25> { static constexpr int R1 = 5, R2 = 5; };
 template <> struct RPlan<14> { static constexpr int R1 = 2, R2 = 7; };
 template <> struct RPlan<50> { static constexpr int R1 = 5, R2 = 10; };
+template <> struct RPlan<40> { static constexpr int R1 = 8, R2 = 5; };
 template <> struct RPlan<36> { static constexpr int R1 = 3, R2 = 12; };
 template <> struct RPlan<28> { static constexpr int R1 = 4, R2 = 7; };
 template <> struct RPlan<20> { static constexpr int R1 = 4, R2 = 5; };
diff --git a/joint-cnn-mrf_amd/csrc/jcm_api.hip b/joint-cnn-mrf_amd/csrc/jcm_api.hip
--- a/joint-cnn-mrf_amd/csrc/jcm_api.hip
+++ b/joint-cnn-mrf_amd/csrc/jcm_api.hip
@@ -275,14 +275,17 @@
   const int np = fft_np(c);
   a.tiles = c->fft_tiles && c->fft_next_pool && !c->fft_t_in && !c->fft_xs && !c->fft_merge && !c->fft_win_map && !circ && in_layout == 0 &&
             np == 4 && conv_fft_tiles_supported(a, L->ks, c->fft_next_ks) ? 1 : 0;
-  const int wH = a.tiles ? H / 2 : H, wW = a.tiles ? W / 2 : W;
+  a.ytiles = c->fft_ytiles && c->fft_fuse == 3 && !c->train && np == 4 && !circ && in_layout == 0 && out_layout == 0 && !c->fft_xs && !c->fft_xs_ready && !c->fft_win_map &&
+             !c->fft_win_scatter && !a.tiles && conv_fft_ytiles_supported(a, L->ks, np) ? 1 : 0;
+  const int wcirc = a.ytiles ? 1 : circ;
+  const int wH = a.tiles ? H / 2 : a.ytiles ? kFftYtileNY : H, wW = a.tiles ? W / 2 : a.ytiles ? 96 : W;
   void* work = arena_alloc<char>(c, conv_fft_workspace_bytes(a, L->ks, np));
   c->arena_off = mark;
   if (c->dry) { c->fft_t_in = nullptr; c->fft_t_next = nullptr; c->fft_merge = nullptr; c->fft_xs = nullptr; c->fft_xs_ready = false; c->fft_tmax_in = nullptr; c->fft_next_pool = 0; c->fft_next_ks = 0; c->fft_next_merge = nullptr; c->fft_t_in_16 = false; c->fft_win_map = nullptr; c->fft_win_scatter = false; return JCM_OK; }
-  const std::string key = scope + (circ ? "@win" : "@") + std::to_string(wH) + "x" + std::to_string(wW);
+  const std::string key = scope + (a.ytiles ? "@ytile" : circ ? "@win" : "@") + std::to_string(wH) + "x" + std::to_string(wW);
   if (!c->fft_w.count(key)) {
     static const size_t cap = [] { const char* e = std::getenv("JCM_FFT_CACHE_GB"); return (size_t)(e ? std::atoi(e) : 64) << 30; }();
-    const size_t need = conv_fft_weight_bytes(wH, wW, L->ks, L->cin, L->cout, np, circ);
+    const size_t need = conv_fft_weight_bytes(wH, wW, L->ks, L->cin, L->cout, np, wcirc);
     size_t held = 0;
     for (auto& kv : c->fft_w) held += kv.second.bytes;
     if (held + need > cap && !c->fft_w.empty()) {
@@ -293,7 +296,7 @@
   }
   jcm_ctx::FftW& fw = c->fft_w[key];
   if (!fw.p) {
-    const size_t wb = (conv_fft_weight_bytes(wH, wW, L->ks, L->cin, L->cout, np, circ) + 255) & ~size_t(255);
+    const size_t wb = (conv_fft_weight_bytes(wH, wW, L->ks, L->cin, L->cout, np, wcirc) + 255) & ~size_t(255);
     fw.bytes = wb + 256;
     if (hipMalloc(&fw.p, fw.bytes) == hipSuccess) {
       fw.wscale = reinterpret_cast<float*>(static_cast<char*>(fw.p) + wb);
@@ -309,7 +312,7 @@
       auto it = c->fft_w.find(key.substr(6));
       if (it != c->fft_w.end() && it->second.valid && it->second.wscale) bound_from = it->second.wscale;
     }
-    HIP_TRY(conv_fft_pack_weights(L->w_raw, fw.p, wH, wW, L->ks, L->cin, L->cout, np, c->precision == JCM_PRECISION_BF16, c->stream, fw.wscale, circ, bound_from));
+    HIP_TRY(conv_fft_pack_weights(L->w_raw, fw.p, wH, wW, L->ks, L->cin, L->cout, np, c->precision == JCM_PRECISION_BF16, c->stream, fw.wscale, wcirc, bound_from));
     fw.valid = true;
   }
   a.wp = fw.p;
@@ -792,6 +795,10 @@
   }
   if (k == "fft_tiles") {
     h->fft_tiles = value != 0;
+    return JCM_OK;
+  }
+  if (k == "fft_ytiles") {
+    h->fft_ytiles = value != 0;
     return JCM_OK;
   }
   if (k == "bf16_hpool") {
diff --git a/joint-cnn-mrf_amd/csrc/kernels.h b/joint-cnn-mrf_amd/csrc/kernels.h
--- a/joint-cnn-mrf_amd/csrc/kernels.h
+++ b/joint-cnn-mrf_amd/csrc/kernels.h
@@ -37,6 +37,7 @@
   int win_B = 0, win_H = 0, win_W = 0, win_TY = 0, win_TX = 0, win_valid_only = 0;
   int wout_H = 0, wout_W = 0, wout_TY = 0, wout_TX = 0;
   int tiles = 0;
+  int ytiles = 0;
   int rows_mfma = 0;
   int hpool = 0;
 };
@@ -82,6 +83,8 @@
 bool conv_fft_win_scatter_supported(int win, int Cout);
 bool conv_fft_pool_fusable(const ConvArgs& a, int ks, int ks_next);
 bool conv_fft_tiles_supported(const ConvArgs& a, int ks, int ks_next);
+constexpr int kFftYtileNY = 40;
+bool conv_fft_ytiles_supported(const ConvArgs& a, int ks, int np);
 size_t conv_fft_pool_handover_bytes(const ConvArgs& a, int ks_next);
 bool conv_fft_merge_fusable(const ConvArgs& a, int ks, int ks_next, const FftMerge& m, bool h16 = false);
 size_t conv_fft_xs_bytes(const ConvArgs& a, int ks, int np);
diff --git a/joint-cnn-mrf_amd/engine.py b/joint-cnn-mrf_amd/engine.py
--- a/joint-cnn-mrf_amd/engine.py
+++ b/joint-cnn-mrf_amd/engine.py
@@ -14,7 +14,7 @@
 
 class Engine:
 
-    def __init__(self, device=0, precision='fp32', n_joints=9, stream=None, f32_conv=None, split_min_wgs=None, micro_batch=None, conv9_fft=None, call_order=None, fft_single=None, fft_t16=None, fft_fuse=None, fft_tiles=None):
+    def __init__(self, device=0, precision='fp32', n_joints=9, stream=None, f32_conv=None, split_min_wgs=None, micro_batch=None, conv9_fft=None, call_order=None, fft_single=None, fft_t16=None, fft_fuse=None, fft_tiles=None, fft_ytiles=None):
         if not torch.cuda.is_available():
             raise RuntimeError('joint-cnn-mrf_amd needs an MI355X (gfx950) GPU; torch.cuda.is_available() is False '
                                'and there is no CPU path')
@@ -47,6 +47,8 @@
             self.set_option('fft_fuse', int(fft_fuse))
         if fft_tiles is not None:
             self.set_option('fft_tiles', int(bool(fft_tiles)))
+        if fft_ytiles is not None:
+            self.set_option('fft_ytiles', int(bool(fft_ytiles)))
         if call_order is not None:
             self.set_option('call_order', int(bool(call_order)))
         if split_min_wgs is not None:
```

Measured after the change: 7159 images/sec, median of 2. No clear change (-0.3%).
